# mandanasmi/lane-slam

Measured on AMD Instinct MI355X. Metric: frames/sec (640x480) detect->descript->project->sanity->associate, higher is better.
Workload: dtype u8/f64 (FP4 e2m1 MFMA with exact f32 accumulation for association)

## Files before the change

### include/lanefront.h

```cpp
#ifndef LANEFRONT_H
#define LANEFRONT_H

#include <stddef.h>
#include <stdint.h>

#define LF_API __attribute__((visibility("default")))

#ifdef __cplusplus
extern "C" {
#endif

#define LF_ABI_VERSION 5

typedef enum lf_status {
    LF_OK = 0,
    LF_ERR_BAD_ARG = -1,
    LF_ERR_CAPACITY = -2,
    LF_ERR_HIP = -3,
    LF_ERR_NOT_INITIALISED = -4,
    LF_ERR_UNSUPPORTED = -5,
    LF_ERR_DECODE = -6
} lf_status;

#define LF_WHITE 0
// ... 66 lines not shown
    double rho, theta;
} lf_hough_params;
LF_API void lf_hough_default_params(lf_hough_params* p);
LF_API int lf_set_hough_params(lf_handle* h, const lf_hough_params* p);
LF_API int lf_get_hough_params(const lf_handle* h, lf_hough_params* p);
#define LF_DETECTOR_DENSE 3
typedef struct lf_dense_params {
    double sobel_threshold;
} lf_dense_params;
LF_API void lf_dense_default_params(lf_dense_params* p);
LF_API int lf_set_dense_params(lf_handle* h, const lf_dense_params* p);
LF_API int lf_get_dense_params(const lf_handle* h, lf_dense_params* p);

#define LF_TIE_LOWEST 0
#define LF_TIE_MIHASHER 1
LF_API int lf_associate(lf_handle* h, const uint8_t* query32, int nq, const uint8_t* map32, int nm,
                 int32_t* idx, float* dist, int on_device);
LF_API int lf_set_tie_rule(lf_handle* h, int tie_rule);
LF_API int lf_associate_float(lf_handle* h, const float* query72, int nq, const float* map72, int nm,
                       int32_t* idx, float* dist, int on_device);

LF_API int lf_knn_match(lf_handle* h, const uint8_t* query32, int nq, const uint8_t* map32, int nm, int k, int32_t* idx, float* dist,
                 int on_device);
LF_API int lf_select_queries(lf_handle* h, const uint8_t* query32, int nq, const uint8_t* mask, uint8_t* selected32, int32_t* query_idx,
                      int* n_selected, int on_device);
LF_API int lf_radius_match(lf_handle* h, const uint8_t* query32, int nq, const uint8_t* map32, int nm, float max_distance,
                    int32_t* offsets, int32_t* idx, float* dist, int cap, int* total, int on_device);

typedef struct { int32_t queryIdx, trainIdx, imgIdx; float distance; } lf_dmatch;
LF_API int lf_matcher_add(lf_handle* h, const uint8_t* codes32, int n, int on_device);
LF_API int lf_matcher_clear(lf_handle* h);
LF_API int lf_matcher_size(const lf_handle* h, int* n_images, int* n_descriptors);
LF_API int lf_matcher_match(lf_handle* h, const uint8_t* query32, int nq, const uint8_t* const* masks, lf_dmatch* out, int* n_out);
LF_API int lf_matcher_knn_match(lf_handle* h, const uint8_t* query32, int nq, int k, const uint8_t* const* masks, int compact_result,
                         int32_t* list_offsets, lf_dmatch* out, int* n_lists);
LF_API int lf_matcher_radius_match(lf_handle* h, const uint8_t* query32, int nq, float max_distance, const uint8_t* const* masks,
                            int compact_result, int32_t* list_offsets, lf_dmatch* out, int cap, int* n_lists, int* total);

LF_API int lf_kmeans(lf_handle* h, const uint8_t* bgr_points, int n, int on_device, int k, const double* init_centers, int max_iter,
              double tol, double* centers_out, long long* counts_out, double* inertia_out, int* n_iter_out);

typedef struct lf_ai_transform {
    int32_t status;
    int32_t success;
    int32_t n_colors;
    int32_t n_iter3, n_iter4;
    int32_t reserved;
    double scale[3], shift[3];
    double cost, health;
    double score3, score4;
    double centers[3][3];
    int64_t counts[3];
} lf_ai_transform;
LF_API int lf_ai_transform_batch(lf_handle* h, const uint8_t* frames, int n_frames, int frames_on_device, int rows, int cols,
                                 lf_ai_transform* out);
LF_API int lf_set_ai_transform(lf_handle* h, const double scale[3], const double shift[3]);
LF_API int lf_get_ai_transform(const lf_handle* h, double scale[3], double shift[3]);

typedef struct lf_map lf_map;
#define LF_MAP_APPEND 0
#define LF_MAP_MERGE 1
#define LF_MAP_RING 0
#define LF_MAP_FULL_ERROR 1
#define LF_BLOCK_ROW_BYTES 80
typedef struct lf_map_config {
    int32_t capacity;
    int32_t color_gating;
    int32_t max_distance;
    int32_t policy;
    int32_t kept_only;
    int32_t merge_distance;
    int32_t when_full;
} lf_map_config;

LF_API int lf_map_create(int device_id, const lf_map_config* cfg, lf_map** out);
LF_API void lf_map_destroy(lf_map* m);
LF_API const char* lf_map_last_error(const lf_map* m);
LF_API int lf_map_get_stream(lf_map* m, void** hip_stream);
LF_API int lf_map_synchronize(lf_map* m);
LF_API int lf_map_seed(lf_map* m, const uint8_t* code32, const uint8_t* color, const double* ground4, int n, int on_device);
LF_API int lf_map_size(lf_map* m, int* size, int* head, int64_t* total_appended, int64_t* total_refreshed);
LF_API int lf_map_associate(lf_map* m, lf_handle* h, const uint8_t* code32, const uint8_t* color, int n,
                     int32_t* idx, float* dist, int on_device);
LF_API int lf_map_set_tie_rule(lf_map* m, int tie_rule);
LF_API int lf_map_pack_block(lf_map* m, lf_handle* h, const lf_segments* segs, int n, int n_frames, const int32_t* idx,
                      const float* dist, const double* frame_pose, int step, uint8_t* block, int block_rows);
LF_API int lf_map_update(lf_map* m, const uint8_t* blocks, int n_blocks, int block_rows);
LF_API int lf_map_step(lf_map* m, lf_handle* h, const lf_segments* segs, int n, int n_frames, const double* frame_pose,
                int step, int32_t* idx, float* dist);
LF_API int lf_map_step_host(lf_map* m, const lf_segments* segs, int n, int n_frames, const double* frame_pose, int step,
                     int32_t* idx, float* dist);
LF_API int lf_map_fetch(lf_map* m, int first, int n, uint8_t* code32, uint8_t* color, double* ground4, int32_t* hits,
                 int32_t* last_seen);

#define LF_MAP_N_STAGES 4
LF_API int lf_map_set_profiling(lf_map* m, int enabled);
LF_API int lf_map_get_timing(lf_map* m, double* ms_per_stage, int32_t* launches_per_stage, int n);
LF_API const char* lf_map_stage_name(int stage);

typedef struct lf_map_view {
    int32_t rows, cols;
    double  x_min, y_max;
    double  pixels_per_metre;
    int32_t thickness;
    int32_t min_hits;
    int32_t min_last_seen;
    uint32_t color_mask;
    uint8_t background[3];
    uint8_t pad_[1];
} lf_map_view;

LF_API void lf_map_default_view(lf_map_view* v);
LF_API int lf_map_bounds(lf_map* m, const lf_map_view* v, double* bounds4, int* n_entries);
LF_API int lf_map_render(lf_map* m, const lf_map_view* v, const double* trajectory, int n_points, uint8_t* out, int out_on_device,
                  int* n_drawn, int* n_skipped);
LF_API int lf_map_render_counts(lf_map* m, int* n_drawn, int* n_skipped);
#define LF_MAP_RENDER_STAGES 4
LF_API int lf_map_render_timing(lf_map* m, double* ms_per_stage, int n);
LF_API const char* lf_map_render_stage_name(int stage);

typedef struct lf_camera_view {
    int32_t rows, cols;
    int32_t top_cutoff;
    int32_t cam_w, cam_h;
    double  hinv[9];
    double  w_near;
    int32_t thickness;
    int32_t min_hits, min_last_seen;
    uint32_t color_mask;
    int32_t palette_size;
    uint8_t palette[8][3];
    uint8_t background[3];
    uint8_t pad_[1];
} lf_camera_view;
LF_API int lf_sizeof_camera_view(void);
LF_API int lf_map_camera_view(const double* H, int cam_w, int cam_h, int rows, int cols, int top_cutoff, lf_camera_view* v);
LF_API int lf_map_render_camera(lf_map* m, const lf_camera_view* v, const double* frame_pose, int n_frames, const uint8_t* src, uint8_t* out,
                         int on_device, int32_t* counts );
LF_API int lf_map_render_camera_timing(lf_map* m, double* ms_per_stage, int n);

typedef struct lf_align_config {
    int32_t iterations;
    int32_t min_pairs;
    int32_t min_hits;
    int32_t color_match;
    double  gate;
    double  huber;
    double  max_dist;
    double  prior_xy, prior_theta;
    double  max_shift, max_turn;
} lf_align_config;
typedef struct lf_align_result {
    double  x, y, theta;
    double  cost0, cost;
    int32_t n_pairs, n_used;
    int32_t iterations;
    int32_t status;
} lf_align_result;
enum { LF_ALIGN_OK = 0, LF_ALIGN_FEW = 1, LF_ALIGN_DEGENERATE = 2, LF_ALIGN_REJECTED = 3 };
LF_API int lf_sizeof_align_config(void);
LF_API int lf_sizeof_align_result(void);
LF_API void lf_map_align_default_config(lf_align_config* c);
LF_API int lf_map_align(lf_map* m, lf_handle* h, const lf_segments* segs, int n, int n_frames, const int32_t* idx, const float* dist,
                 const double* frame_pose , const lf_align_config* cfg, int on_device,
                 lf_align_result* results );
LF_API int lf_map_step_aligned(lf_map* m, lf_handle* h, const lf_segments* segs, int n, int n_frames, const double* frame_pose,
// ... 266 lines not shown
LF_API int lf_get_descriptor_params(lf_handle* h, lf_descriptor_params* p);
LF_API int lf_keylines_batch(lf_handle* h, const uint8_t* images, int n_frames, int input_kind, int images_on_device, int n_octaves,
                      const lf_edlines_params* params_or_null, lf_keylines* out, int out_on_device, int describe,
                      int* n_keylines, int32_t* frame_status_or_null);
LF_API int lf_keylines_batch_masked(lf_handle* h, const uint8_t* images, int n_frames, int input_kind, int images_on_device, int n_octaves,
                             const lf_edlines_params* params_or_null, const uint8_t* masks, int masks_on_device, lf_keylines* out,
                             int out_on_device, int describe, int* n_keylines, int32_t* frame_status);
LF_API int lf_keylines_batch_async(lf_handle* h, const uint8_t* images_dev, int n_frames, int input_kind, int n_octaves,
                            const lf_edlines_params* params_or_null, lf_keylines* out_dev, int describe);
LF_API int lf_keylines_frame_status(lf_handle* h, int32_t* frame_status, int n_frames);
LF_API int lf_lsd_keylines_batch(lf_handle* h, const uint8_t* images, int n_frames, int input_kind, int images_on_device, int n_octaves,
                          lf_keylines* out, int out_on_device, int describe, int* n_keylines);
typedef struct {
    int32_t refine;
    int32_t n_bins;
    double scale, sigma_scale, quant, ang_th, log_eps, density_th;
    double min_length;
} lf_lsd_options;
LF_API void lf_lsd_default_options(lf_lsd_options* opts);
LF_API int lf_lsd_keylines_batch_ex(lf_handle* h, const uint8_t* images, int n_frames, int input_kind, int images_on_device, int n_octaves,
                             const lf_lsd_options* opts, const uint8_t* masks, int masks_on_device,
                             lf_keylines* out, int out_on_device, int describe, int* n_keylines);
LF_API int lf_set_image_edlines(lf_handle* h, const uint8_t* bgr, int rows, int cols, int row_stride_bytes,
                         const lf_edlines_params* params_or_null);
LF_API int lf_describe_keylines(lf_handle* h, const uint8_t* gray, int n_frames, const int32_t* line_frame, const float* in_octave4,
                         const float* angle, const int32_t* num_pixels, const int32_t* octave, int n, float* desc72,
                         uint8_t* code32, int on_device);
LF_API int lf_keylines_debug_fetch(lf_handle* h, int octave, int what, void* dst, size_t bytes, int32_t* dims5_or_null);

LF_API int lf_jpeg_decode_batch(lf_handle* h, const uint8_t* const* jpeg, const size_t* jpeg_size, int n_frames,
                         int rows, int cols, uint8_t* frames, int frames_on_device, int n_threads,
                         int* frame_status);
LF_API int lf_jpeg_decode_batch_gpu(lf_handle* h, const uint8_t* const* jpeg, const size_t* jpeg_size, int n_frames,
                             int rows, int cols, uint8_t* frames, int frames_on_device, int n_threads,
                             int* frame_status);
LF_API int lf_jpeg_decode_batch_gpu_async(lf_handle* h, const uint8_t* const* jpeg, const size_t* jpeg_size, int n_frames,
                                   int rows, int cols, uint8_t* frames_device, int n_threads);
LF_API int lf_jpeg_status(lf_handle* h, int* frame_status, int n_frames, int* n_failed);
LF_API int lf_jpeg_decode_for_detect_async(lf_handle* h, const uint8_t* const* jpeg, const size_t* jpeg_size, int n_frames, int n_threads);
LF_API int lf_jpeg_info(const uint8_t* jpeg, size_t jpeg_size, int* rows, int* cols, int* components, int* hmax, int* vmax);
LF_API int lf_frames_buffer(lf_handle* h, uint8_t** device_ptr, size_t* bytes);

#define LF_MSG_DETECTOR 0
#define LF_MSG_GROUND 1
#define LF_MSG_FILTERED 2
LF_API int lf_serialize_segments(lf_handle* h, const lf_segments* segs, int segs_on_device, int n_frames, int stage,
                          uint8_t* out, size_t out_capacity, int out_on_device, int64_t* frame_byte_offset);
LF_API int lf_deserialize_segments(lf_handle* h, const uint8_t* bodies, int bodies_on_device, const int64_t* frame_byte_offset,
                            int n_frames, lf_segments* out, int out_on_device, int* n_segments);

LF_API int lf_draw_lines(lf_handle* h, int n_frames, const lf_segments* seg, int seg_on_device, uint8_t* out_bgr, int out_on_device);
LF_API int lf_draw_lines_image(lf_handle* h, const uint8_t* bgr, int n_frames, int rows, int cols, const lf_segments* seg, int seg_on_device,
                               uint8_t* out_bgr, int images_on_device);

#define LF_JPEG_ENCODE_STAGES 8
LF_API size_t lf_jpeg_encode_bound(int rows, int cols);
LF_API int lf_jpeg_encode_batch(lf_handle* h, const uint8_t* bgr, int bgr_on_device, int n_frames, int rows, int cols, int quality, uint8_t* out,
                                size_t out_stride, uint32_t* out_size, int out_on_device);
LF_API int lf_jpeg_encode_timing(lf_handle* h, double* ms_per_stage, int n);
LF_API const char* lf_jpeg_encode_stage_name(int stage);

#define LF_RECTIFY_STAGES 1
LF_API int lf_set_camera(lf_handle* h, const double* K, const double* D, const double* R, const double* P, int cam_w, int cam_h);
LF_API int lf_set_rectified_input(lf_handle* h, int flag);
LF_API int lf_get_rectified_input(lf_handle* h, int* flag);
LF_API int lf_rectify_map(lf_handle* h, float* mapx, float* mapy);
LF_API int lf_rectify_batch(lf_handle* h, const uint8_t* src, int src_on_device, int n_frames, int rows, int cols, int channels, uint8_t* dst,
                            int dst_on_device);
LF_API int lf_rectify_timing(lf_handle* h, double* ms_per_stage, int n);
LF_API const char* lf_rectify_stage_name(int stage);

typedef enum lf_buffer_id {
    LF_BUF_BGR = 0,
    LF_BUF_MASKS = 1,
    LF_BUF_EDGES = 2,
    LF_BUF_LSD_ANGLE = 3,
    LF_BUF_LSD_MODGRAD = 4,
    LF_BUF_LSD_ORDER = 5,
    LF_BUF_LSD_NORDER = 6,
    LF_BUF_LBD_DX = 7,
    LF_BUF_LBD_DY = 8,
    LF_BUF_LSD_COUNTS = 9,
    LF_BUF_LSD_SCRATCH = 10,
    LF_BUF_LSD_NLOW = 11
} lf_buffer_id;
LF_API int lf_debug_fetch(lf_handle* h, int buffer_id, void* dst, size_t bytes);
LF_API int lf_debug_detmath(lf_handle* h, int which, const double* a, const double* b_or_null, double* y, int n);
enum { LF_WAVE_INT = 0, LF_WAVE_UINT = 1, LF_WAVE_FLOAT = 2, LF_WAVE_DOUBLE = 3, LF_WAVE_LONG = 4, LF_WAVE_ULONG = 5 };
enum {
    LF_WAVE_READLANE = 0, LF_WAVE_DPP = 1, LF_WAVE_SUM = 2, LF_WAVE_MAX = 3, LF_WAVE_MIN = 4, LF_WAVE_INCL_SCAN_DPP = 5,
    LF_WAVE_INCL_MIN_DPP = 6, LF_WAVE_SUM_BCAST = 7, LF_WAVE_MIN_BCAST = 8, LF_WAVE_INCL_SCAN = 9, LF_WAVE_REDUCE = 10,
    LF_WAVE_BALLOT = 11, LF_WAVE_LANE_MASK_LT = 12, LF_WAVE_LANES_BELOW = 13, LF_WAVE_BALLOT_BRANCH = 14, LF_WAVE_UNI = 15,
    LF_WAVE_WG_EXCL_SCAN = 16, LF_WAVE_WG_SCAN_TURNS = 17
};
LF_API int lf_debug_wave(lf_handle* h, int op, int type, int arg, int diverge, const uint64_t* in, uint64_t* out, int n_threads, int block);
LF_API int lf_debug_probe(lf_handle* h, int width, int write, size_t bytes, int reps);
LF_API int lf_debug_lsd_binary(lf_handle* h, const uint8_t* img, int rows, int cols, float* lines4, int cap, int* n_out);
LF_API int lf_debug_hysteresis(lf_handle* h, const uint8_t* planes_u8, int n_frames, int rows, int cols, uint8_t* edges_u8_out);
LF_API int lf_debug_segments(lf_handle* h, int mode, int n_frames, const int32_t* counts, const float* lines4, const uint8_t* masks,
                             lf_segments* out, int* n_segments);
LF_API int lf_debug_std_sort(lf_handle* h, const int32_t* keys, int n, int32_t* order);
LF_API int lf_debug_assoc_plan(int nq, int nm, int32_t out[6]);
LF_API int lf_lsd_size(const lf_handle* h, int* rows, int* cols);
LF_API int lf_suggested_depth(const lf_handle* h);

LF_API int lf_lsd_list_capacity(const lf_handle* h, int* entries, int* grown);
LF_API int lf_lsd_scratch_stride(const lf_handle* h);

#define LF_N_STAGES 16
LF_API int lf_set_profiling(lf_handle* h, int enabled);
LF_API int lf_get_timing(lf_handle* h, double* ms_per_stage, int32_t* launches_per_stage, int n);
LF_API int lf_reset_timing(lf_handle* h);
LF_API const char* lf_stage_name(int stage);

#ifdef __cplusplus
}
#endif
#endif
```

### lane_slam_amd/_lib.py

```python
import ctypes
import os

from .config import LfConfig

_HERE = os.path.dirname(os.path.abspath(__file__))
SO_PATH = os.environ.get("LANEFRONT_LIBRARY") or os.path.join(_HERE, "liblanefront.so")

LF_N_STAGES = 16
LF_MAP_N_STAGES = 4
LF_MSG_DETECTOR, LF_MSG_GROUND, LF_MSG_FILTERED = 0, 1, 2
(LF_BUF_BGR, LF_BUF_MASKS, LF_BUF_EDGES, LF_BUF_LSD_ANGLE, LF_BUF_LSD_MODGRAD, LF_BUF_LSD_ORDER,
 LF_BUF_LSD_NORDER, LF_BUF_LBD_DX, LF_BUF_LBD_DY, LF_BUF_LSD_COUNTS, LF_BUF_LSD_SCRATCH, LF_BUF_LSD_NLOW) = range(12)

EXPORTS = (
    "lf_abi_version", "lf_create", "lf_destroy", "lf_last_error", "lf_synchronize", "lf_get_stream",
    "lf_set_image", "lf_detect_lines", "lf_process_batch", "lf_process_batch_async", "lf_wait", "lf_associate", "lf_associate_float", "lf_kmeans",
    "lf_jpeg_decode_batch", "lf_jpeg_info", "lf_frames_buffer", "lf_serialize_segments", "lf_deserialize_segments",
    "lf_debug_fetch", "lf_debug_detmath", "lf_debug_wave", "lf_debug_probe", "lf_debug_lsd_binary", "lf_debug_segments", "lf_debug_hysteresis", "lf_lsd_size", "lf_set_profiling", "lf_get_timing", "lf_reset_timing", "lf_stage_name",
    "lf_map_create", "lf_map_destroy", "lf_map_last_error", "lf_map_get_stream", "lf_map_synchronize", "lf_map_seed", "lf_map_size",
    "lf_map_associate", "lf_map_pack_block", "lf_map_update", "lf_map_step", "lf_map_step_host", "lf_map_fetch",
    "lf_map_set_profiling", "lf_map_get_timing", "lf_map_stage_name",
    "lf_descriptor_default_params", "lf_set_descriptor_params", "lf_get_descriptor_params",
    "lf_edlines_default_params", "lf_keylines_batch", "lf_describe_keylines", "lf_keylines_debug_fetch", "lf_set_image_edlines", "lf_knn_match", "lf_radius_match", "lf_jpeg_decode_batch_gpu", "lf_jpeg_decode_batch_gpu_async", "lf_jpeg_status", "lf_jpeg_decode_for_detect_async",
    "lf_set_tie_rule", "lf_map_set_tie_rule", "lf_debug_std_sort", "lf_debug_assoc_plan", "lf_suggested_depth", "lf_lsd_list_capacity", "lf_lsd_scratch_stride", "lf_set_detector", "lf_detector_failures", "lf_keylines_batch_async", "lf_keylines_frame_status", "lf_lsd_keylines_batch", "lf_select_queries",
    "lf_lsd_default_options", "lf_lsd_keylines_batch_ex", "lf_keylines_batch_masked",
    "lf_matcher_add", "lf_matcher_clear", "lf_matcher_size", "lf_matcher_match", "lf_matcher_knn_match", "lf_matcher_radius_match",
    "lf_lane_filter_default_config", "lf_lane_filter_create", "lf_lane_filter_destroy", "lf_lane_filter_last_error", "lf_lane_filter_grid",
    "lf_lane_filter_set_tables", "lf_lane_filter_reset", "lf_lane_filter_step", "lf_lane_filter_get_poses", "lf_lane_filter_get_belief",
    "lf_lane_filter_synchronize", "lf_lane_filter_set_profiling", "lf_lane_filter_get_timing", "lf_lane_filter_stage_name",
    "lf_hough_default_params", "lf_set_hough_params", "lf_get_hough_params",
    "lf_dense_default_params", "lf_set_dense_params", "lf_get_dense_params",
    "lf_ai_transform_batch", "lf_set_ai_transform", "lf_get_ai_transform",
    "lf_draw_lines", "lf_draw_lines_image",
    "lf_jpeg_encode_bound", "lf_jpeg_encode_batch", "lf_jpeg_encode_timing", "lf_jpeg_encode_stage_name",
    "lf_set_camera", "lf_set_rectified_input", "lf_get_rectified_input", "lf_rectify_map", "lf_rectify_batch", "lf_rectify_timing",
    "lf_rectify_stage_name",
    "lf_map_default_view", "lf_map_bounds", "lf_map_render", "lf_map_render_counts", "lf_map_render_timing", "lf_map_render_stage_name",
    "lf_sizeof_camera_view", "lf_map_camera_view", "lf_map_render_camera", "lf_map_render_camera_timing",
    "lf_sizeof_align_config", "lf_sizeof_align_result", "lf_map_align_default_config", "lf_map_align", "lf_map_step_aligned",
    "lf_map_step_aligned_host", "lf_map_align_timing",
    "lf_sizeof_smooth_config", "lf_map_smooth_default_config", "lf_map_smooth", "lf_map_step_smoothed", "lf_map_step_smoothed_host",
    "lf_map_smooth_timing",
    "lf_sizeof_localize_config", "lf_sizeof_localize_result", "lf_map_localize_default_config", "lf_map_localize", "lf_map_localize_timing",
    "lf_sizeof_prune_config", "lf_sizeof_prune_result", "lf_map_prune_default_config", "lf_map_prune", "lf_map_prune_timing",
    "lf_sizeof_near_config", "lf_map_near_default_config", "lf_map_associate_near", "lf_map_set_near", "lf_map_get_near", "lf_map_near_timing",
    "lf_sizeof_lanes_config", "lf_sizeof_lane", "lf_sizeof_lanes_result", "lf_map_lanes_default_config", "lf_map_lanes", "lf_map_lanes_timing",
    "lf_sizeof_polylines_config", "lf_sizeof_polyline_vertex", "lf_sizeof_polyline", "lf_sizeof_polylines_result",
    "lf_map_polylines_default_config", "lf_map_polylines", "lf_map_polylines_timing",
    "lf_sizeof_lane_pose_config", "lf_sizeof_lane_pose", "lf_sizeof_lane_pose_result",
    "lf_map_lane_pose_default_config", "lf_map_lane_pose", "lf_map_lane_pose_timing",
    "lf_sizeof_graph_config", "lf_sizeof_graph_result", "lf_map_graph_default_config", "lf_map_graph_solve", "lf_map_correct",
    "lf_map_graph_timing",
)
LF_ALIGN_OK, LF_ALIGN_FEW, LF_ALIGN_DEGENERATE, LF_ALIGN_REJECTED = 0, 1, 2, 3
ALIGN_STATUS = ("ok", "few", "degenerate", "rejected")
LF_MAP_RENDER_STAGES = 4
LF_JPEG_ENCODE_STAGES = 8
LF_RECTIFY_STAGES = 1
LF_LANE_FILTER_PREDICT, LF_LANE_FILTER_UPDATE = 1, 2
LF_LANE_FILTER_MAX_CELLS = 4096
LF_LANE_FILTER_N_STAGES = 2
LANE_FILTER_PARAMS = ("mean_d_0", "mean_phi_0", "sigma_d_0", "sigma_phi_0", "delta_d", "delta_phi", "d_max", "d_min", "phi_max",
                      "phi_min", "cov_v", "linewidth_white", "linewidth_yellow", "lanewidth", "min_max", "sigma_d_mask", "sigma_phi_mask")
DETECTORS = {"lsd": 0, "edlines": 1, "hough": 2, "dense": 3}
HOUGH_KEYS = ("hough_threshold", "hough_min_line_length", "hough_max_line_gap")
DENSE_KEYS = ("sobel_threshold",)
TIE_RULES = {"lowest": 0, "mihasher": 1}
LF_MAX_OCTAVES = 5


class LfSegments(ctypes.Structure):
    _fields_ = [
        ("capacity", ctypes.c_int32),
        ("frame_offset", ctypes.c_void_p),
        ("lines", ctypes.c_void_p), ("normals", ctypes.c_void_p), ("color", ctypes.c_void_p),
        ("pixels_normalized", ctypes.c_void_p), ("ground", ctypes.c_void_p), ("keep", ctypes.c_void_p),
        ("desc", ctypes.c_void_p), ("code", ctypes.c_void_p),
    ]


class LfEdlinesParams(ctypes.Structure):
    _fields_ = [("gradient_threshold", ctypes.c_int32), ("anchor_threshold", ctypes.c_int32), ("scan_intervals", ctypes.c_int32),
                ("min_line_len", ctypes.c_int32), ("line_fit_err_threshold", ctypes.c_double), ("ksize", ctypes.c_int32)]


class LfHoughParams(ctypes.Structure):
    _fields_ = [("threshold", ctypes.c_int32), ("min_line_length", ctypes.c_int32), ("max_line_gap", ctypes.c_int32),
                ("rho", ctypes.c_double), ("theta", ctypes.c_double)]


class LfDenseParams(ctypes.Structure):
    _fields_ = [("sobel_threshold", ctypes.c_double)]


class LfAiTransform(ctypes.Structure):
    _fields_ = [("status", ctypes.c_int32), ("success", ctypes.c_int32), ("n_colors", ctypes.c_int32), ("n_iter3", ctypes.c_int32),
                ("n_iter4", ctypes.c_int32), ("reserved", ctypes.c_int32), ("scale", ctypes.c_double * 3), ("shift", ctypes.c_double * 3),
                ("cost", ctypes.c_double), ("health", ctypes.c_double), ("score3", ctypes.c_double), ("score4", ctypes.c_double),
                ("centers", ctypes.c_double * 9), ("counts", ctypes.c_int64 * 3)]


class LfDescriptorParams(ctypes.Structure):
    _fields_ = [("num_of_octave", ctypes.c_int32), ("width_of_band", ctypes.c_int32), ("reduction_ratio", ctypes.c_int32), ("ksize", ctypes.c_int32)]

# ... 211 lines not shown
    lib.lf_get_ai_transform.argtypes = [vp, vp, vp]
    lib.lf_draw_lines.argtypes = [vp, ci, ctypes.POINTER(LfSegments), ci, vp, ci]
    lib.lf_draw_lines_image.argtypes = [vp, vp, ci, ci, ci, ctypes.POINTER(LfSegments), ci, vp, ci]
    lib.lf_jpeg_encode_bound.argtypes = [ci, ci]
    lib.lf_jpeg_encode_bound.restype = ctypes.c_size_t
    lib.lf_jpeg_encode_batch.argtypes = [vp, vp, ci, ci, ci, ci, ci, vp, ctypes.c_size_t, vp, ci]
    lib.lf_jpeg_encode_batch.restype = ci
    lib.lf_jpeg_encode_timing.argtypes = [vp, vp, ci]
    lib.lf_jpeg_encode_timing.restype = ci
    lib.lf_jpeg_encode_stage_name.argtypes = [ci]
    lib.lf_jpeg_encode_stage_name.restype = ctypes.c_char_p
    lib.lf_set_camera.argtypes = [vp, vp, vp, vp, vp, ci, ci]
    lib.lf_set_rectified_input.argtypes = [vp, ci]
    lib.lf_get_rectified_input.argtypes = [vp, ctypes.POINTER(ci)]
    lib.lf_rectify_map.argtypes = [vp, vp, vp]
    lib.lf_rectify_batch.argtypes = [vp, vp, ci, ci, ci, ci, ci, vp, ci]
    lib.lf_rectify_timing.argtypes = [vp, vp, ci]
    for f in ("lf_set_camera", "lf_set_rectified_input", "lf_get_rectified_input", "lf_rectify_map", "lf_rectify_batch", "lf_rectify_timing"):
        getattr(lib, f).restype = ci
    lib.lf_rectify_stage_name.argtypes = [ci]
    lib.lf_rectify_stage_name.restype = ctypes.c_char_p
    lib.lf_jpeg_decode_batch.argtypes = [vp, ctypes.POINTER(vp), ctypes.POINTER(ctypes.c_size_t), ci, ci, ci, vp, ci, ci,
                                         ctypes.POINTER(ci)]
    lib.lf_jpeg_decode_batch.restype = ci
    lib.lf_jpeg_decode_batch_gpu.argtypes = lib.lf_jpeg_decode_batch.argtypes
    lib.lf_jpeg_decode_batch_gpu.restype = ci
    lib.lf_jpeg_decode_batch_gpu_async.argtypes = [vp, ctypes.POINTER(vp), ctypes.POINTER(ctypes.c_size_t), ci, ci, ci, vp, ci]
    lib.lf_jpeg_decode_batch_gpu_async.restype = ci
    lib.lf_jpeg_status.argtypes = [vp, ctypes.POINTER(ci), ci, ctypes.POINTER(ci)]
    lib.lf_jpeg_decode_for_detect_async.argtypes = [vp, ctypes.POINTER(vp), ctypes.POINTER(ctypes.c_size_t), ci, ci]
    lib.lf_jpeg_decode_for_detect_async.restype = ci
    lib.lf_jpeg_status.restype = ci
    lib.lf_jpeg_info.argtypes = [vp, ctypes.c_size_t] + [ctypes.POINTER(ci)] * 5
    lib.lf_jpeg_info.restype = ci
    lib.lf_frames_buffer.argtypes = [vp, ctypes.POINTER(vp), ctypes.POINTER(ctypes.c_size_t)]
    lib.lf_frames_buffer.restype = ci
    lib.lf_serialize_segments.argtypes = [vp, ctypes.POINTER(LfSegments), ci, ci, ci, vp, ctypes.c_size_t, ci,
                                          ctypes.POINTER(ctypes.c_int64)]
    lib.lf_serialize_segments.restype = ci
    lib.lf_deserialize_segments.argtypes = [vp, vp, ci, ctypes.POINTER(ctypes.c_int64), ci, ctypes.POINTER(LfSegments), ci,
                                            ctypes.POINTER(ci)]
    lib.lf_deserialize_segments.restype = ci
    lib.lf_debug_fetch.argtypes = [vp, ci, vp, ctypes.c_size_t]
    lib.lf_debug_detmath.argtypes = [vp, ci, vp, vp, vp, ci]
    lib.lf_debug_detmath.restype = ci
    lib.lf_debug_wave.argtypes = [vp, ci, ci, ci, ci, vp, vp, ci, ci]
    lib.lf_debug_wave.restype = ci
    lib.lf_debug_probe.argtypes = [vp, ci, ci, ctypes.c_size_t, ci]
    lib.lf_debug_probe.restype = ci
    lib.lf_debug_lsd_binary.argtypes = [vp, vp, ci, ci, vp, ci, ctypes.POINTER(ci)]
    lib.lf_debug_lsd_binary.restype = ci
    lib.lf_debug_segments.argtypes = [vp, ci, ci, vp, vp, vp, ctypes.POINTER(LfSegments), ctypes.POINTER(ci)]
    lib.lf_debug_hysteresis.argtypes = [vp, vp, ci, ci, ci, vp]
    lib.lf_debug_hysteresis.restype = ci
    lib.lf_lsd_size.argtypes = [vp, ctypes.POINTER(ci), ctypes.POINTER(ci)]
    lib.lf_set_profiling.argtypes = [vp, ci]
    lib.lf_get_timing.argtypes = [vp, vp, vp, ci]
    lib.lf_reset_timing.argtypes = [vp]
    lib.lf_stage_name.argtypes = [ci]
    lib.lf_stage_name.restype = ctypes.c_char_p
    i64p = ctypes.POINTER(ctypes.c_int64)
    lib.lf_map_create.argtypes = [ci, ctypes.POINTER(LfMapConfig), ctypes.POINTER(vp)]
    lib.lf_map_destroy.argtypes = [vp]
    lib.lf_map_destroy.restype = None
    lib.lf_map_last_error.argtypes = [vp]
    lib.lf_map_last_error.restype = ctypes.c_char_p
    lib.lf_map_get_stream.argtypes = [vp, ctypes.POINTER(vp)]
    lib.lf_map_synchronize.argtypes = [vp]
    lib.lf_map_seed.argtypes = [vp, vp, vp, vp, ci, ci]
    lib.lf_map_size.argtypes = [vp, ctypes.POINTER(ci), ctypes.POINTER(ci), i64p, i64p]
    lib.lf_map_associate.argtypes = [vp, vp, vp, vp, ci, vp, vp, ci]
    lib.lf_map_pack_block.argtypes = [vp, vp, ctypes.POINTER(LfSegments), ci, ci, vp, vp, vp, ci, vp, ci]
    lib.lf_map_update.argtypes = [vp, vp, ci, ci]
    lib.lf_map_step.argtypes = [vp, vp, ctypes.POINTER(LfSegments), ci, ci, vp, ci, vp, vp]
    lib.lf_map_step_host.argtypes = [vp, ctypes.POINTER(LfSegments), ci, ci, vp, ci, vp, vp]
    lib.lf_map_step_host.restype = ci
    lib.lf_map_fetch.argtypes = [vp, ci, ci, vp, vp, vp, vp, vp]
    lib.lf_map_set_profiling.argtypes = [vp, ci]
    lib.lf_map_set_profiling.restype = ci
    lib.lf_map_get_timing.argtypes = [vp, vp, vp, ci]
    lib.lf_map_get_timing.restype = ci
    lib.lf_map_stage_name.argtypes = [ci]
    lib.lf_map_stage_name.restype = ctypes.c_char_p
    lib.lf_map_default_view.argtypes = [ctypes.POINTER(LfMapView)]
    lib.lf_map_default_view.restype = None
    lib.lf_map_bounds.argtypes = [vp, ctypes.POINTER(LfMapView), vp, ctypes.POINTER(ci)]
    lib.lf_map_render.argtypes = [vp, ctypes.POINTER(LfMapView), vp, ci, vp, ci, ctypes.POINTER(ci), ctypes.POINTER(ci)]
    lib.lf_map_render_counts.argtypes = [vp, ctypes.POINTER(ci), ctypes.POINTER(ci)]
    lib.lf_map_render_timing.argtypes = [vp, vp, ci]
    for f in ("lf_map_bounds", "lf_map_render", "lf_map_render_counts", "lf_map_render_timing"):
        getattr(lib, f).restype = ci
    lib.lf_map_render_stage_name.argtypes = [ci]
    lib.lf_map_render_stage_name.restype = ctypes.c_char_p
    lib.lf_sizeof_camera_view.argtypes = []
    lib.lf_map_camera_view.argtypes = [vp, ci, ci, ci, ci, ci, ctypes.POINTER(LfCameraView)]
    lib.lf_map_render_camera.argtypes = [vp, ctypes.POINTER(LfCameraView), vp, ci, vp, vp, ci, vp]
    lib.lf_map_render_camera_timing.argtypes = [vp, vp, ci]
    for f in ("lf_sizeof_camera_view", "lf_map_camera_view", "lf_map_render_camera", "lf_map_render_camera_timing"):
        getattr(lib, f).restype = ci
    lib.lf_sizeof_align_config.argtypes = []
    lib.lf_sizeof_align_result.argtypes = []
    lib.lf_map_align_default_config.argtypes = [ctypes.POINTER(LfAlignConfig)]
    lib.lf_map_align_default_config.restype = None
    lib.lf_map_align.argtypes = [vp, vp, ctypes.POINTER(LfSegments), ci, ci, vp, vp, vp, ctypes.POINTER(LfAlignConfig), ci, vp]
    lib.lf_map_step_aligned.argtypes = [vp, vp, ctypes.POINTER(LfSegments), ci, ci, vp, ctypes.POINTER(LfAlignConfig), ci, vp, vp, vp]
    lib.lf_map_step_aligned_host.argtypes = [vp, ctypes.POINTER(LfSegments), ci, ci, vp, ctypes.POINTER(LfAlignConfig), ci, vp, vp, vp]
    lib.lf_map_align_timing.argtypes = [vp, ctypes.POINTER(ctypes.c_double), ctypes.POINTER(ctypes.c_int32)]
    for f in ("lf_sizeof_align_config", "lf_sizeof_align_result", "lf_map_align", "lf_map_step_aligned", "lf_map_step_aligned_host",
              "lf_map_align_timing"):
        getattr(lib, f).restype = ci
    lib.lf_sizeof_smooth_config.argtypes = []
    lib.lf_map_smooth_default_config.argtypes = [ctypes.POINTER(LfSmoothConfig)]
    lib.lf_map_smooth_default_config.restype = None
    lib.lf_map_smooth.argtypes = [vp, vp, ctypes.POINTER(LfSegments), ci, ci, vp, vp, vp, vp, ci, ctypes.POINTER(LfSmoothConfig), ci, vp, vp]
    lib.lf_map_step_smoothed.argtypes = [vp, vp, ctypes.POINTER(LfSegments), ci, ci, vp, vp, ci, ctypes.POINTER(LfSmoothConfig), ci, vp, vp, vp, vp]
    lib.lf_map_step_smoothed_host.argtypes = [vp, ctypes.POINTER(LfSegments), ci, ci, vp, vp, ci, ctypes.POINTER(LfSmoothConfig), ci, vp, vp, vp, vp]
    lib.lf_map_smooth_timing.argtypes = [vp, ctypes.POINTER(ctypes.c_double), ctypes.POINTER(ctypes.c_int32)]
    for f in ("lf_sizeof_smooth_config", "lf_map_smooth", "lf_map_step_smoothed", "lf_map_step_smoothed_host", "lf_map_smooth_timing"):
        getattr(lib, f).restype = ci
    lib.lf_sizeof_localize_config.argtypes = []
    lib.lf_sizeof_localize_result.argtypes = []
    lib.lf_map_localize_default_config.argtypes = [ctypes.POINTER(LfLocalizeConfig)]
    lib.lf_map_localize_default_config.restype = None
    lib.lf_map_localize.argtypes = [vp, vp, ctypes.POINTER(LfSegments), ci, ci, vp, vp, vp, ctypes.POINTER(LfLocalizeConfig), ci, vp]
    lib.lf_map_localize_timing.argtypes = [vp, ctypes.POINTER(ctypes.c_double), ctypes.POINTER(ctypes.c_int32)]
    for f in ("lf_sizeof_localize_config", "lf_sizeof_localize_result", "lf_map_localize", "lf_map_localize_timing"):
        getattr(lib, f).restype = ci
    lib.lf_sizeof_prune_config.argtypes = []
    lib.lf_sizeof_prune_result.argtypes = []
    lib.lf_map_prune_default_config.argtypes = [ctypes.POINTER(LfPruneConfig)]
    lib.lf_map_prune_default_config.restype = None
    lib.lf_map_prune.argtypes = [vp, ctypes.POINTER(LfPruneConfig), ctypes.POINTER(LfPruneResult), vp, ci]
    lib.lf_map_prune_timing.argtypes = [vp, ctypes.POINTER(ctypes.c_double), ctypes.POINTER(ctypes.c_int32)]
    for f in ("lf_sizeof_prune_config", "lf_sizeof_prune_result", "lf_map_prune", "lf_map_prune_timing"):
        getattr(lib, f).restype = ci
    lib.lf_sizeof_near_config.argtypes = []
    lib.lf_map_near_default_config.argtypes = [ctypes.POINTER(LfNearConfig)]
    lib.lf_map_near_default_config.restype = None
    lib.lf_map_associate_near.argtypes = [vp, vp, ctypes.POINTER(LfSegments), ci, ci, vp, ctypes.POINTER(LfNearConfig), vp, vp, vp, ci]
    lib.lf_map_set_near.argtypes = [vp, ctypes.POINTER(LfNearConfig)]
    lib.lf_map_get_near.argtypes = [vp, ctypes.POINTER(LfNearConfig)]
    lib.lf_map_near_timing.argtypes = [vp, ctypes.POINTER(ctypes.c_double), ctypes.POINTER(ctypes.c_int32)]
    for f in ("lf_sizeof_near_config", "lf_map_associate_near", "lf_map_set_near", "lf_map_get_near", "lf_map_near_timing"):
        getattr(lib, f).restype = ci
    for f in ("lf_sizeof_lanes_config", "lf_sizeof_lane", "lf_sizeof_lanes_result"):
        getattr(lib, f).argtypes = []
    lib.lf_map_lanes_default_config.argtypes = [ctypes.POINTER(LfLanesConfig)]
    lib.lf_map_lanes_default_config.restype = None
    lib.lf_map_lanes.argtypes = [vp, ctypes.POINTER(LfLanesConfig), ctypes.POINTER(LfLanesResult), vp, vp, vp, vp, ci, ci]
    lib.lf_map_lanes_timing.argtypes = [vp, ctypes.POINTER(ctypes.c_double), ctypes.POINTER(ctypes.c_int32)]
    for f in ("lf_sizeof_lanes_config", "lf_sizeof_lane", "lf_sizeof_lanes_result", "lf_map_lanes", "lf_map_lanes_timing"):
        getattr(lib, f).restype = ci
    for f in ("lf_sizeof_polylines_config", "lf_sizeof_polyline_vertex", "lf_sizeof_polyline", "lf_sizeof_polylines_result"):
        getattr(lib, f).argtypes = []
        getattr(lib, f).restype = ci
    lib.lf_map_polylines_default_config.argtypes = [ctypes.POINTER(LfPolylinesConfig)]
    lib.lf_map_polylines_default_config.restype = None
    lib.lf_map_polylines.argtypes = [vp, ctypes.POINTER(LfPolylinesConfig), ctypes.POINTER(LfPolylinesResult), vp, vp, ci, vp, ci, ci]
    lib.lf_map_polylines.restype = ci
    lib.lf_map_polylines_timing.argtypes = [vp, ctypes.POINTER(ctypes.c_double), ctypes.POINTER(ctypes.c_int32)]
    lib.lf_map_polylines_timing.restype = ci
    for f in ("lf_sizeof_lane_pose_config", "lf_sizeof_lane_pose", "lf_sizeof_lane_pose_result"):
        getattr(lib, f).argtypes = []
        getattr(lib, f).restype = ci
    lib.lf_map_lane_pose_default_config.argtypes = [ctypes.POINTER(LfLanePoseConfig)]
    lib.lf_map_lane_pose_default_config.restype = None
# ... 120 lines not shown
```

### lane_slam_amd/csrc/common.h

```cpp
#pragma once
#include <hip/hip_runtime.h>
#include <stdint.h>
#include <stddef.h>
#include "../../include/lanefront.h"
#include "detmath.h"

namespace lf {

constexpr int kMaxKsize = 9;
constexpr int kMaxGaussTaps = 15;
constexpr float kNotDef = -1024.0f;
#ifndef LF_LABEL_ITEMS
#define LF_LABEL_ITEMS 8192
#endif
constexpr int kLabelItems = LF_LABEL_ITEMS;
#ifndef LF_LABEL_LDS
#define LF_LABEL_LDS 6144
#endif
constexpr int kLabelLds = LF_LABEL_LDS;
constexpr int kCompCap = 1024;

enum Stage {
    ST_PRE = 0, ST_CANNY, ST_HYST, ST_LSD_GRAD, ST_LSD_ORDER, ST_LSD_GROW, ST_SEGMENTS,
    ST_LBD_GRAD, ST_LBD, ST_ASSOC_PACK, ST_ASSOC, ST_MISC, ST_JPEG, ST_LSD_LABEL, ST_HOUGH, ST_DENSE, ST_COUNT
// ... 223 lines not shown
{
    *reinterpret_cast<uint32_t*>(mx + assoc_map_offset_fp4(pos, 4 * b)) = 0u;
    if (b < 8) *reinterpret_cast<uint32_t*>(mcx + pos * 32 + 4 * b) = 0u;
}
#endif
template <typename T>
struct DevArray {
    T* p = nullptr;
    size_t bytes = 0;
    DevArray() = default;
    DevArray(DevArray&& o) noexcept : p(o.p), bytes(o.bytes) { o.p = nullptr; o.bytes = 0; }
    DevArray& operator=(DevArray&& o) noexcept
    {
        if (this != &o) { reset(); p = o.p; bytes = o.bytes; o.p = nullptr; o.bytes = 0; }
        return *this;
    }
    ~DevArray() { reset(); }
    hipError_t alloc(size_t n_bytes)
    {
        reset();
        const hipError_t e = hipMalloc((void**)&p, n_bytes);
        if (e != hipSuccess) p = nullptr; else bytes = n_bytes;
        return e;
    }
    void reset() { if (p) (void)hipFree(p); p = nullptr; bytes = 0; }
    operator T*() const { return p; }
};
using DevBuf = DevArray<void>;

template <typename T>
struct HostArray {
    T* p = nullptr;
    size_t bytes = 0;
    HostArray() = default;
    HostArray(HostArray&& o) noexcept : p(o.p), bytes(o.bytes) { o.p = nullptr; o.bytes = 0; }
    HostArray& operator=(HostArray&& o) noexcept
    {
        if (this != &o) { reset(); p = o.p; bytes = o.bytes; o.p = nullptr; o.bytes = 0; }
        return *this;
    }
    ~HostArray() { reset(); }
    hipError_t alloc(size_t n_bytes)
    {
        reset();
        const hipError_t e = hipHostMalloc((void**)&p, n_bytes, hipHostMallocDefault);
        if (e != hipSuccess) p = nullptr; else bytes = n_bytes;
        return e;
    }
    void reset() { if (p) (void)hipHostFree(p); p = nullptr; bytes = 0; }
    operator T*() const { return p; }
};

struct AssocScratch {
    DevArray<unsigned int> part; DevArray<int> done; size_t cap_part = 0, cap_blocks = 0;
    int qblocks = 0, splits = 0, m_chunk = 0;
    DevArray<int> tie_list; size_t cap_list = 0;
    unsigned long long* tie_res = nullptr;
};
void launch_assoc_pack_map(const uint8_t* codes, int n, int n_pad, int8_t* x, hipStream_t s);
hipError_t launch_assoc_core(const uint8_t* q, const uint8_t* qcolor, int nq, const int8_t* mx, const int8_t* mcx, int nm,
                             const int* nm_dev, int gating, int max_distance, AssocScratch& w, int32_t* idx, float* dist, hipStream_t s);
hipError_t launch_assoc_ties(const uint8_t* q, const uint8_t* qcolor, int nq, const int8_t* mx, const uint8_t* mcode, const uint8_t* mcolor,
                             int nm, const int* nm_dev, int gating, AssocScratch& w, unsigned long long* res, int32_t* idx, const float* dist, hipStream_t s);
hipError_t launch_assoc(const uint8_t* q, int nq, const uint8_t* m, int nm, int8_t* mx, AssocScratch& w, int32_t* idx, float* dist, hipStream_t s);
void launch_assoc_nomatch(int nq, int32_t* idx, float* dist, hipStream_t s);
void launch_kmeans(const uint8_t* bgr, int n, int k, const double* init, int max_iter, double tol_rel, uint8_t* lab, double* out,
                   long long* counts, int* status, hipStream_t s);
void launch_draw(const void* src, bool src_bgrx, uint8_t* out, int n_frames, int Hc, int W, const int32_t* frame_offset, const float* lines,
                 const uint8_t* color, int capacity, int* bad, hipStream_t s);
void launch_ai_transform(const uint8_t* strips, long long frame_stride, int n_frames, int S, int cols, uint8_t* lab, double* fo,
                         long long* fc, int* fs, lf_ai_transform* out, hipStream_t s);
struct MapDevice {
    int capacity, policy, kept_only, merge_distance, when_full;
    uint8_t* code; uint8_t* color; double* ground; int* hits; int* last_seen; int* winner;
    int8_t* mx; int8_t* mcx;
    int* state;
    unsigned long long* totals;
};
void launch_fill_i32(int* p, size_t n, int v, hipStream_t s);
void launch_map_pack_block(int n, int n_frames, const int* frame_offset, const uint8_t* code, const uint8_t* color,
                           const uint8_t* keep, const double* ground, const int32_t* idx, const float* dist,
                           const double* pose4, int step, uint8_t* block, hipStream_t s);
void launch_map_overflow_block(int n, int n_frames, int step, uint8_t* block, hipStream_t s);
void launch_map_seed_block(int n, const uint8_t* code, const uint8_t* color, const double* ground, uint8_t* block, hipStream_t s);
void launch_map_update(const MapDevice& md, const uint8_t* blocks, int n_blocks, int block_rows, int force_append, int* act,
                       hipStream_t s);
void launch_select_queries(const uint8_t* q, const uint8_t* mask, int nq, uint8_t* out, int32_t* qidx, int* n_out, hipStream_t s);
void launch_knn(const uint8_t* q, int nq, const uint8_t* m, int nm, int k, int max_distance, int mih, int32_t* idx, float* dist, hipStream_t s);
void launch_radius(const uint8_t* q, int nq, const uint8_t* m, int nm, int max_distance, int32_t* hist, int32_t* count, int32_t* offsets,
                   int* total, int cap, int mih, int32_t* idx, float* dist, hipStream_t s);
size_t assoc_float_scratch_bytes(int nq, int nm);
hipError_t launch_assoc_float(const float* q, int nq, const float* m, int nm, float* qn, float* mn,
                              void* scratch, int32_t* idx, float* dist, hipStream_t s);
namespace jpeg { struct FrameHeader; }
struct JpegGeom { int rows, cols, Wp, Hp; int first_row = 0; };
void launch_jpeg_decode(const JpegGeom& g, int n_frames, int max_blocks, const jpeg::FrameHeader* hdrs,
                        const uint32_t* entries, const uint32_t* block_end, uint8_t* planes, uint8_t* frames,
                        hipStream_t s);

void launch_jpeg_color(const JpegGeom& g, int n_frames, const void* hdrs, size_t hdr_stride, const uint8_t* planes, uint8_t* frames, hipStream_t s);
namespace jpeg { struct DevFrame; }
void launch_jh_decode(const JpegGeom& g, int n_frames, int max_blocks, size_t max_scan_len, jpeg::DevFrame* frames, const uint8_t* bytes, uint8_t* clean,
                      uint32_t* seg_begin, void* info, uint32_t* sub, int16_t* coef, int* status, uint8_t* planes, hipStream_t s);
size_t jh_info_bytes();

void launch_msg_layout(int n_frames, int stage, const int* frame_offset, const uint8_t* keep, int* counts,
                       long long* byte_offset, hipStream_t s);
void launch_msg_write(int n_frames, int stage, const int* frame_offset, const uint8_t* color, const float* pixels_normalized,
                      const float* normals, const double* ground, const uint8_t* keep, const int* counts,
                      const long long* byte_offset, uint8_t* out, hipStream_t s);
void launch_msg_read(int n_frames, int capacity, const uint8_t* body, const long long* byte_offset, int* frame_offset,
                     int* bad, uint8_t* color, float* pixels_normalized, float* normals, double* ground, hipStream_t s);

}
```

### lane_slam_amd/csrc/k_lsd_order.hip

```cpp
#include <cstdlib>
#include <algorithm>
#include "common.h"
#include <type_traits>
#include "lsd_bitplane.h"
#include "scan.h"
#include "wave.h"

namespace lf {
using std::max;
using std::min;

#ifndef LF_ORDER_THREADS
#define LF_ORDER_THREADS 512
#endif
#ifndef LF_ORDER_BM_THREADS
#define LF_ORDER_BM_THREADS 256
#endif
#ifndef LF_LABEL_THREADS
#define LF_LABEL_THREADS 256
#endif
constexpr int OT = LF_ORDER_THREADS;
constexpr int OBT = LF_ORDER_BM_THREADS;
constexpr int NB = 16;
constexpr int LDS_ITEMS = 8192;
// ... 501 lines not shown
        __syncthreads();
    } else {
        for (int e = t; e < n; e += LT) reinterpret_cast<uint16_t*>(dyn_lds + LS / 2)[e] = (uint16_t)(c_xy[o + e] & 0xffffu);
        __syncthreads();
    for (int e = t; e < n; e += LT) {
        const int y = (int)(c_xy[o + e] >> 16);
        const int first = rs[y];
        int h = e;
        int xh = xs(h);
        while (h > first) { const int xp = xs(h - 1); if (xp + 1 != xh) break; --h; xh = xp; }
        parent.set((uint32_t)e, (uint32_t)h);
    }
    __syncthreads();
    for (int e = t; e < n; e += LT) {
        const uint32_t xy = c_xy[o + e];
        const int x = (int)(xy & 0xffffu), y = (int)(xy >> 16);
        if (y > 0) {
            int lo = rs[y - 1];
            const int end = rs[y];
            int hi = end;
            while (lo < hi) { const int mid = (lo + hi) >> 1; if (xs(mid) < x - 1) lo = mid + 1; else hi = mid; }
            for (int k = lo; k < end && k < lo + 3 && xs(k) <= x + 1; ++k) uf_unite(parent, (uint32_t)e, (uint32_t)k);
        }
    }
    __syncthreads();
    }
    for (int i = t; i < (n + 1) / 2; i += LT) csize2.set((uint32_t)i, 0u);
    __syncthreads();
    for (int e = t; e < n; e += LT) {
        const uint32_t r = uf_find(parent, (uint32_t)e);
        lab[e] = (uint16_t)r;
        csize2.add(r >> 1, 1u << (16 * (r & 1u)));
    }
    __syncthreads();
    auto csize = [&](uint32_t r) -> uint32_t { return (csize2.get(r >> 1) >> (16 * (r & 1u))) & 0xffffu; };
    const uint32_t minsz = p.min_reg_size > 1 ? (uint32_t)p.min_reg_size : 1u;
    for (int e = t; e < n; e += LT)
        if (csize((uint32_t)e) >= minsz) {
            const int k = atomicAdd(&n_roots, 1);
            if (k < comp_cap) roots[k] = (uint16_t)e;
        }
    __syncthreads();
    const int C = n_roots;
    if (C > comp_cap) {
        for (int e = t; e < n; e += LT) lab[e] = 0;
        if (t == 0) { list[0] = 0; comp_count[pc] = 1; comp_key[pc] = n; }
        return;
    }
    for (int i = t; i < C; i += LT) {
        const uint32_t ri = roots[i], si = csize(ri);
        int rank = 0;
        for (int j = 0; j < C; ++j) {
            const uint32_t rj = roots[j], sj = csize(rj);
            rank += (sj > si || (sj == si && rj < ri)) ? 1 : 0;
        }
        list[rank] = (uint16_t)ri;
        parent.set(ri, (uint32_t)rank);
        if (rank == 0) comp_key[pc] = (int)si;
        if (rank >= kCompTop) atomicAdd(&rest_total, (int)si);
    }
    __syncthreads();
    if (C <= kCompTop) {
        if (t == 0) { comp_count[pc] = C; if (C == 0) comp_key[pc] = 0; }
        return;
    }
    __threadfence_block();
    const uint16_t rest_root = list[kCompTop];
    for (int e = t; e < n; e += LT) {
        const uint32_t r = lab[e];
        if (csize(r) >= minsz && parent.get(r) >= (uint32_t)kCompTop) lab[e] = rest_root;
    }
    if (t == 0) {
        const int rest = rest_total;
        const int top0 = (int)csize((uint32_t)list[0]);
        if (rest > top0) {
            for (int k = kCompTop; k > 0; --k) list[k] = list[k - 1];
            list[0] = rest_root;
            comp_key[pc] = rest;
        }
        comp_count[pc] = kCompTop + 1;
    }
}

__global__ __launch_bounds__(256) void k_lsd_rank(int n_prob, const int* __restrict__ norder, int* __restrict__ perm)
{
    __shared__ int nd[1024];
    if (n_prob > 1024) {
        for (int i = threadIdx.x; i < n_prob; i += 256) perm[i] = i;
        return;
    }
    for (int i = threadIdx.x; i < n_prob; i += 256) nd[i] = norder[i];
    __syncthreads();
    for (int i = threadIdx.x; i < n_prob; i += 256) {
        const int mine = nd[i];
        int rank = 0;
        for (int j = 0; j < n_prob; ++j) rank += (nd[j] > mine || (nd[j] == mine && j < i)) ? 1 : 0;
        perm[rank] = i;
    }
}

void launch_lsd_rank(const LsdComponents& m, int n_prob, hipStream_t s)
{
    hipLaunchKernelGGL(k_lsd_rank, dim3(1), dim3(256), 0, s, n_prob, m.comp_key, m.perm);
}

__global__ __launch_bounds__(LT) void k_lsd_label(LsdParams p, const int* __restrict__ norder, const uint32_t* __restrict__ c_xy,
                                                  const int* __restrict__ row_start, uint16_t* __restrict__ c_label,
                                                  uint16_t* __restrict__ comp_list, int* __restrict__ comp_count, int* __restrict__ comp_key, int comp_cap,
                                                  uint32_t* __restrict__ scratch, size_t scratch_stride, int plane_fits)
{
    const int n = norder[blockIdx.x];
    if (n <= p.label_lds)
        lsd_label_problem<false>(p, norder, c_xy, row_start, c_label, comp_list, comp_count, comp_key, comp_cap, scratch, scratch_stride);
    else if (plane_fits)
        lsd_label_problem<true>(p, norder, c_xy, row_start, c_label, comp_list, comp_count, comp_key, comp_cap, scratch, scratch_stride);
    else {
        const size_t o = (size_t)blockIdx.x * p.rec_cap;
        for (int e = threadIdx.x; e < n; e += LT) c_label[o + e] = 0;
        if (threadIdx.x == 0) { comp_list[(size_t)blockIdx.x * kCompCap] = 0; comp_count[blockIdx.x] = 1; comp_key[blockIdx.x] = n; }
    }
}

void launch_lsd_label(const LsdParams& p, const LsdCompact& c, const LsdComponents& m, int n_frames, hipStream_t s)
{
    size_t lds = (size_t)p.label_lds * (2 + 2);
    const size_t plane = bitplane_lds_words((size_t)p.Hs * p.Ws) * 4;
    const int plane_fits = plane <= 150 * 1024 ? 1 : 0;
    if (plane_fits && plane > lds) lds = plane;
    if (lds > 48 * 1024)
        (void)hipFuncSetAttribute(reinterpret_cast<const void*>(k_lsd_label), hipFuncAttributeMaxDynamicSharedMemorySize, (int)lds);
    static const int comp_cap = getenv("LF_DIAG_COMP_CAP") ? max(1, min(kCompCap, atoi(getenv("LF_DIAG_COMP_CAP")))) : kCompCap;
    const size_t stride = lsd_grow_reg_stride(p);
    hipLaunchKernelGGL(k_lsd_label, dim3(n_frames * 3), dim3(LT), lds, s, p, c.norder, c.c_xy, c.row_start, m.c_label, m.comp_list, m.comp_count,
                       m.comp_key, comp_cap, m.reg, stride, plane_fits);
}

__global__ void k_lsd_dense_debug(LsdParams p, const int* __restrict__ norder, const uint32_t* __restrict__ c_xy,
                                  const float* __restrict__ c_deg, const double* __restrict__ c_mod,
                                  float* __restrict__ ang, double* __restrict__ mod)
{
    const int pc = blockIdx.x;
    const size_t Ps = (size_t)p.Hs * p.Ws, o = (size_t)pc * Ps, oc = (size_t)pc * p.rec_cap;
    for (size_t i = threadIdx.x; i < Ps; i += blockDim.x) { ang[o + i] = kNotDef; mod[o + i] = 0.0; }
    __syncthreads();
    const int n = norder[pc];
    for (int e = threadIdx.x; e < n; e += blockDim.x) {
        const uint32_t xy = c_xy[oc + e];
        const size_t a = (size_t)(xy >> 16) * p.Ws + (xy & 0xffffu);
        ang[o + a] = c_deg[oc + e];
        mod[o + a] = c_mod[oc + e];
    }
}

void launch_lsd_dense_debug(const LsdParams& p, const LsdCompact& c, int n_frames, float* ang, double* mod, hipStream_t s)
{
    hipLaunchKernelGGL(k_lsd_dense_debug, dim3(n_frames * 3), dim3(1024), 0, s, p, c.norder, c.c_xy, c.c_deg, c.c_mod, ang, mod);
}

}
```

### lane_slam_amd/csrc/k_map.hip

```cpp
#include "common.h"
#include "scan.h"

namespace lf {

constexpr int kRow = LF_BLOCK_ROW_BYTES;
constexpr int kRefFlag = 0x40000000;
constexpr uint32_t kMagic = 0x4b42464cu;

struct MapDev {
    int capacity, policy, kept_only, merge_distance, when_full;
    uint8_t* code; uint8_t* color; double* ground; int* hits; int* last_seen; int* winner;
    int8_t* mx; int8_t* mcx;
    int* state;
    unsigned long long* totals;
};

__global__ void k_map_pack_block(int n, int n_frames, const int* __restrict__ frame_offset, const uint8_t* __restrict__ code,
                                 const uint8_t* __restrict__ color, const uint8_t* __restrict__ keep,
                                 const double* __restrict__ ground, const int32_t* __restrict__ idx,
                                 const float* __restrict__ dist, const double* __restrict__ pose4, int step,
                                 uint8_t* __restrict__ block)
{
    const int s = blockIdx.x * blockDim.x + threadIdx.x;
    if (s == 0) {
// ... 126 lines not shown
    const int s = (int)(t >> 5), b = (int)(t & 31);
    if ((size_t)s >= total) return;
    int a = act[s];
    if (a == -1) return;
    if (!(a & kRefFlag)) a += wg_base[s / kMapWg];
    const int n_app = m.state[3], head0 = m.state[5], size0 = m.state[6], step = m.state[7];
    const int cap = m.capacity;
    int pos;
    bool fresh;
    if (a & kRefFlag) {
        pos = a & ~kRefFlag;
        if (m.winner[pos] != s) return;
        bool overwritten = false;
        if (m.when_full == LF_MAP_RING) {
            int rel = pos - head0; if (rel < 0) rel += cap;
            overwritten = n_app >= cap || rel < n_app;
        }
        if (overwritten) { if (b == 0) m.winner[pos] = -1; return; }
        fresh = false;
    } else {
        if (m.when_full == LF_MAP_RING) {
            if (n_app > cap && a < n_app - cap) return;
            pos = (int)(((long long)head0 + a) % cap);
        } else {
            if (a >= cap - size0) return;
            pos = size0 + a;
        }
        fresh = true;
    }
    const int blk = s / G, r = s - blk * G;
    const uint8_t* row = blocks + ((size_t)blk * block_rows + 1 + r) * kRow;
    const uint32_t byte = row[b];
    m.code[(size_t)pos * 32 + b] = (uint8_t)byte;
    assoc_map_write_row(m.mx, m.mcx, (size_t)pos, b, byte, row + 72);
    if (b == 0) {
        m.color[pos] = row[72];
        const double* rg = reinterpret_cast<const double*>(row + 32);
        for (int k = 0; k < 4; ++k) m.ground[(size_t)pos * 4 + k] = rg[k];
        m.last_seen[pos] = step;
        if (fresh) m.hits[pos] = 1; else m.winner[pos] = -1;
    }
}

__global__ void k_map_seed_block(int n, const uint8_t* __restrict__ code, const uint8_t* __restrict__ color,
                                 const double* __restrict__ ground, uint8_t* __restrict__ block)
{
    const int s = blockIdx.x * blockDim.x + threadIdx.x;
    if (s == 0) {
        uint32_t* hd = reinterpret_cast<uint32_t*>(block);
        hd[0] = kMagic; hd[1] = (uint32_t)n; hd[2] = (uint32_t)-1; hd[3] = 0u;
        for (int k = 4; k < kRow / 4; ++k) hd[k] = 0u;
    }
    if (s >= n) return;
    uint8_t* row = block + (size_t)(1 + s) * kRow;
    for (int k = 0; k < 32; ++k) row[k] = code[(size_t)s * 32 + k];
    double* rg = reinterpret_cast<double*>(row + 32);
    for (int k = 0; k < 4; ++k) rg[k] = ground ? ground[(size_t)s * 4 + k] : 0.0;
    *reinterpret_cast<int32_t*>(row + 64) = -1;
    *reinterpret_cast<float*>(row + 68) = -1.f;
    row[72] = color ? color[s] : (uint8_t)255;
    row[73] = 1;
    row[74] = row[75] = row[76] = row[77] = row[78] = row[79] = 0;
}

__global__ void k_fill_i32(int* p, size_t n, int v)
{
    for (size_t i = blockIdx.x * (size_t)blockDim.x + threadIdx.x; i < n; i += (size_t)gridDim.x * blockDim.x) p[i] = v;
}

void launch_fill_i32(int* p, size_t n, int v, hipStream_t s)
{
    if (n) hipLaunchKernelGGL(k_fill_i32, dim3(1024), dim3(256), 0, s, p, n, v);
}

void launch_map_pack_block(int n, int n_frames, const int* frame_offset, const uint8_t* code, const uint8_t* color,
                           const uint8_t* keep, const double* ground, const int32_t* idx, const float* dist,
                           const double* pose4, int step, uint8_t* block, hipStream_t s)
{
    const int threads = n > 0 ? n : 1;
    hipLaunchKernelGGL(k_map_pack_block, dim3((threads + 255) / 256), dim3(256), 0, s, n, n_frames, frame_offset, code, color,
                       keep, ground, idx, dist, pose4, step, block);
}

__global__ void k_map_overflow_block(int n, int n_frames, int step, uint8_t* __restrict__ block)
{
    uint32_t* hd = reinterpret_cast<uint32_t*>(block);
    const int k = threadIdx.x;
    if (k < kRow / 4) hd[k] = k == 0 ? kMagic : k == 2 ? (uint32_t)step : k == 3 ? (uint32_t)n_frames : k == 4 ? (uint32_t)n : 0u;
}

void launch_map_overflow_block(int n, int n_frames, int step, uint8_t* block, hipStream_t s)
{
    hipLaunchKernelGGL(k_map_overflow_block, dim3(1), dim3(64), 0, s, n, n_frames, step, block);
}

void launch_map_seed_block(int n, const uint8_t* code, const uint8_t* color, const double* ground, uint8_t* block, hipStream_t s)
{
    const int threads = n > 0 ? n : 1;
    hipLaunchKernelGGL(k_map_seed_block, dim3((threads + 255) / 256), dim3(256), 0, s, n, code, color, ground, block);
}

void launch_map_update(const MapDevice& md, const uint8_t* blocks, int n_blocks, int block_rows, int force_append, int* act,
                       hipStream_t s)
{
    MapDev m;
    m.capacity = md.capacity; m.policy = md.policy; m.kept_only = md.kept_only; m.merge_distance = md.merge_distance;
    m.when_full = md.when_full;
    m.code = md.code; m.color = md.color; m.ground = md.ground; m.hits = md.hits; m.last_seen = md.last_seen;
    m.winner = md.winner; m.mx = md.mx; m.mcx = md.mcx; m.state = md.state; m.totals = md.totals;
    const size_t rows = (size_t)n_blocks * (block_rows - 1);
    const int n_wg = (int)((rows + kMapWg - 1) / kMapWg);
    int* wg_count = act + rows;
    if (n_wg)
        hipLaunchKernelGGL(k_map_classify, dim3(n_wg), dim3(kMapWg), 0, s, m, blocks, n_blocks, block_rows, force_append, act, wg_count);
    hipLaunchKernelGGL(k_map_plan, dim3(1), dim3(kMapWg), 0, s, m, blocks, n_blocks, n_wg, wg_count);
    const size_t threads = rows * 32;
    if (threads)
        hipLaunchKernelGGL(k_map_apply, dim3((threads + 255) / 256), dim3(256), 0, s, m, blocks, n_blocks, block_rows, act, wg_count);
}

}
```

### lane_slam_amd/csrc/lanefront_api.hip

```cpp
#include <stdarg.h>
#include <stdio.h>
#include <string.h>
#include <math.h>
#include <vector>
#include <new>
#include <cstdlib>
#include "lanefront_handle.h"

using namespace lf;

static const char* kStageNames[LF_N_STAGES] = {
    "pre(resize+correct+hsv+masks+dilate)", "canny_nms", "canny_hysteresis", "lsd_blur_resample_grad",
    "lsd_order", "lsd_grow", "segments(normal+project+sanity)", "lbd_gray_blur_sobel", "lbd_descriptor",
    "assoc_pack", "assoc_mfma", "misc", "jpeg(idct+upsample+color)", "lsd_label(components+launch order)",
    "hough(probabilistic lines)", "dense(sobel-vote lines)" };

extern "C" void lf_set_error(lf_handle* h, int code, const char* fmt, ...)
{
    va_list ap;
    va_start(ap, fmt);
    vset_error(h, code, fmt, ap);
    va_end(ap);
}

static char g_create_err[512] = "no error";

static int cv_round_host(double v) { return dm::round_half_even(v); }

static int build_params(lf_handle* h)
{
    const lf_config& c = h->cfg;
    h->Hc = c.img_rows - c.top_cutoff;
    h->W = c.img_cols;
    if (h->Hc <= 0 || h->W <= 0 || c.in_rows <= 0 || c.in_cols <= 0 || c.top_cutoff < 0) {
        lf_set_error(h, LF_ERR_BAD_ARG, "bad geometry: in %dx%d img %dx%d cutoff %d", c.in_rows, c.in_cols, c.img_rows,
                     c.img_cols, c.top_cutoff);
        return LF_ERR_BAD_ARG;
    }
    if (h->W % 32 != 0) { lf_set_error(h, LF_ERR_UNSUPPORTED, "img_cols must be a multiple of 32 (got %d)", h->W); return LF_ERR_UNSUPPORTED; }
    h->P = (size_t)h->Hc * h->W;
    h->Ww = (h->W + 31) / 32;
    PreParams& p = h->pre;
    memset(&p, 0, sizeof(p));
    p.in_rows = c.in_rows; p.in_cols = c.in_cols; p.img_rows = c.img_rows; p.img_cols = c.img_cols;
    p.top_cutoff = c.top_cutoff; p.Hc = h->Hc; p.W = h->W;
    p.resize = (c.img_rows != c.in_rows) || (c.img_cols != c.in_cols);
    const double fx = (double)c.img_cols / (double)c.in_cols, fy = (double)c.img_rows / (double)c.in_rows;
    p.ifx = 1.0 / fx; p.ify = 1.0 / fy;
    p.identity_ai = 1;
    for (int i = 0; i < 3; ++i) { p.ai_scale[i] = c.ai_scale[i]; p.ai_shift[i] = c.ai_shift[i]; if (c.ai_scale[i] != 1.f || c.ai_shift[i] != 0.f) p.identity_ai = 0; }
    for (int k = 0; k < 4; ++k) for (int ch = 0; ch < 3; ++ch) { p.lo[k][ch] = c.hsv_lo[k][ch]; p.hi[k][ch] = c.hsv_hi[k][ch]; }
    p.ksize = c.dilation_kernel_size;
    if (p.ksize < 1 || p.ksize > kMaxKsize) { lf_set_error(h, LF_ERR_UNSUPPORTED, "dilation_kernel_size %d not in [1,%d]", p.ksize, kMaxKsize); return LF_ERR_UNSUPPORTED; }
    p.r = p.ksize / 2;
    {
        int r = p.ksize / 2, cc = p.ksize / 2;
        double inv_r2 = r ? 1.0 / ((double)r * r) : 0.0;
        for (int i = 0; i < p.ksize; ++i) {
            int dy = i - r;
            p.j1[i] = 0; p.j2[i] = 0;
            if (abs(dy) <= r) {
                int dx = cv_round_host(cc * sqrt((r * r - dy * dy) * inv_r2));
                p.j1[i] = cc - dx > 0 ? cc - dx : 0;
                p.j2[i] = cc + dx + 1 < p.ksize ? cc + dx + 1 : p.ksize;
            }
        }
        if (p.ksize % 2 == 0) { lf_set_error(h, LF_ERR_UNSUPPORTED, "even dilation kernels are not supported"); return LF_ERR_UNSUPPORTED; }
    }
    h->canny.Hc = h->Hc; h->canny.W = h->W; h->canny.Ww = h->Ww;
    double lo = c.canny_lo, hi = c.canny_hi;
    if (lo > hi) { double t = lo; lo = hi; hi = t; }
    h->canny.low = dm::ifloor(lo); h->canny.high = dm::ifloor(hi);
    if ((size_t)h->Hc * h->Ww > 8 * 1024 && (8192 / h->Ww < 1 || (int)((60 * 1024 / 4) / (2 * (size_t)h->Ww)) - 1 < 1)) { lf_set_error(h, LF_ERR_UNSUPPORTED, "img_cols %d: one row of the edge bit planes exceeds the hysteresis strip budget", h->W); return LF_ERR_UNSUPPORTED; }
    SegParams& S = h->seg;
    memset(&S, 0, sizeof(S));
    S.Hc = h->Hc; S.W = h->W; S.img_rows = c.img_rows; S.img_cols = c.img_cols; S.top_cutoff = c.top_cutoff;
    S.cap_lines = h->cap_lines;
    S.rx = 1.0 / (double)c.img_cols; S.ry = 1.0 / (double)c.img_rows; S.cut = (double)c.top_cutoff;
    memcpy(S.H, c.H, sizeof(S.H));
    seg_camera(h);
    S.lanewidth = c.lanewidth; S.linewidth_white = c.linewidth_white; S.linewidth_yellow = c.linewidth_yellow;
    S.d_min = c.d_min; S.d_max = c.d_max; S.phi_min = c.phi_min; S.phi_max = c.phi_max;
    return LF_OK;
}

static int lbd_weights(lf_handle* h, int w)
// ... 198 lines not shown
            return LF_ERR_UNSUPPORTED;
        }
    }
    if (h->detector == LF_DETECTOR_HOUGH) {
        int rc = hough_prepare(h);
        if (rc != LF_OK) return rc;
        StageClock::Scope t(h, h->clock, ST_HOUGH);
        LF_HIP_CHECK(h, hipMemsetAsync(h->lsd.d_zero, 0, h->lsd.zero_bytes, s));
        HoughParams hp = h->hough_p;
        hp.threshold = h->hough_params.threshold; hp.line_length = h->hough_params.min_line_length; hp.line_gap = h->hough_params.max_line_gap;
        launch_hough(hp, n * 3, h->hough_slots < n * 3 ? h->hough_slots : n * 3, h->d_strong, h->d_maskbits, h->d_hough_tab, h->d_hough_acc,
                     h->d_hough_nz, h->d_slot_lines, h->d_counts, s);
        LF_HIP_CHECK(h, hipGetLastError());
        h->slot_mode = SEG_HOUGH;
        h->last_frames = n;
        h->overflow_zeroed = true;
        return LF_OK;
    }
    if (dense) {
        StageClock::Scope t(h, h->clock, ST_DENSE);
        LF_HIP_CHECK(h, hipMemsetAsync(h->lsd.d_zero, 0, h->lsd.zero_bytes, s));
        launch_dense(h->Hc, h->W, h->Ww, h->cap_lines, (float)h->dense_params.sobel_threshold, n * 3, h->d_strong, h->d_maskbits,
                     h->d_bwbits, h->d_slot_lines, h->d_dense_rec, h->d_counts, s);
        LF_HIP_CHECK(h, hipGetLastError());
        h->slot_mode = SEG_DENSE;
        h->last_frames = n;
        h->overflow_zeroed = true;
        return LF_OK;
    }
    h->slot_mode = SEG_FLOAT;
    {
        StageClock::Scope t(h, h->clock, ST_LSD_GRAD);
        LF_HIP_CHECK(h, hipMemsetAsync(h->lsd.d_zero, 0, h->lsd.zero_bytes, s));
        h->lsd.grad(n, h->d_strong, h->d_maskbits, true, s);
    }
    { StageClock::Scope t(h, h->clock, ST_LSD_ORDER); h->lsd.order(n, 0, s); }
    {
        StageClock::Scope t(h, h->clock, ST_LSD_LABEL);
        h->lsd.label(n, true, s);
    }
    static const char* diag_skip = getenv("LF_DIAG_SKIP");
    if (diag_skip && strstr(diag_skip, "grow")) LF_HIP_CHECK(h, hipMemsetAsync(h->d_counts, 0, (size_t)n * 3 * sizeof(int), s));
    else {
        StageClock::Scope t(h, h->clock, ST_LSD_GROW);
        const LsdState& L = h->lsd;
        h->lsd.grow(n, h->d_slot_lines, h->d_counts, kGrowLdsKb[L.env_lds_level >= 0 ? L.env_lds_level : L.grow_lds_level],
                    L.env_mixed >= 0 ? L.env_mixed != 0 : L.grow_mixed, true, s);
    }
    LF_HIP_CHECK(h, hipGetLastError());
    h->last_frames = n;
    h->overflow_zeroed = true;
    return LF_OK;
}

int lf::run_segments(lf_handle* h, int n, lf_segments dev_out, bool describe)
{
    hipStream_t s = h->stream;
    {
        StageClock::Scope t(h, h->clock, ST_SEGMENTS);
        if (!h->overflow_zeroed) LF_HIP_CHECK(h, hipMemsetAsync(h->lsd.d_status, 0, offsetof(BatchStatus, detector_failures), s));
        h->overflow_zeroed = false;
        launch_seg_offsets(n, h->cap_lines, h->d_counts, h->d_seg_offset, dev_out.frame_offset ? dev_out.frame_offset : h->d_frame_offset,
                           h->lsd.d_status, h->slot_mode != SEG_FLOAT ? nullptr : h->lsd.d_norder, lsd_grow_def_lds(h->lsd.params, kGrowLdsKb[0]),
                           lsd_grow_def_lds(h->lsd.params, kGrowLdsKb[1]), s);
        launch_segments(h->seg, n, h->d_slot_lines, h->d_counts, h->d_seg_offset,
                        h->slot_mode == SEG_DENSE ? reinterpret_cast<const uint32_t*>(h->d_dense_rec.p) : h->d_maskbits.p, h->Ww, dev_out,
                        h->d_seg_frame, h->d_normals64, h->d_centers, s, h->slot_mode);
    }
    if (describe) {
        { StageClock::Scope t(h, h->clock, ST_LBD_GRAD); launch_lbd_grad(h->Hc, h->W, n, h->d_gray, h->d_dxy, s); }
        {
            StageClock::Scope t(h, h->clock, ST_LBD);
            int cap = dev_out.capacity < n * 3 * h->cap_lines ? dev_out.capacity : n * 3 * h->cap_lines;
            launch_lbd(h->Hc, h->W, cap, h->d_seg_offset + n * 3, dev_out.lines, h->d_seg_frame, h->d_dxy,
                       h->d_gauss_g, h->d_gauss_l, dev_out.desc, dev_out.code, s, h->desc_params.width_of_band);
        }
    }
    LF_HIP_CHECK(h, hipGetLastError());
    return LF_OK;
}

static int fetch_status(lf_handle* h) { LF_HIP_CHECK(h, hipMemcpyAsync(h->h_status, h->lsd.d_status, sizeof(BatchStatus), hipMemcpyDeviceToHost, h->stream)); return LF_OK; }

extern "C" int lf_process_batch_async(lf_handle* h, const uint8_t* frames, int n_frames, int frames_on_device,
                                      lf_segments* out_dev, int describe)
{
    if (!h) return LF_ERR_NOT_INITIALISED;
    if (!frames || !out_dev || n_frames < 1) { lf_set_error(h, LF_ERR_BAD_ARG, "lf_process_batch: null argument or n_frames < 1"); return LF_ERR_BAD_ARG; }
    if (n_frames > h->max_frames) { lf_set_error(h, LF_ERR_CAPACITY, "n_frames %d exceeds max_frames %d", n_frames, h->max_frames); return LF_ERR_CAPACITY; }
    if (describe && (!out_dev->lines)) { lf_set_error(h, LF_ERR_BAD_ARG, "describe needs out->lines"); return LF_ERR_BAD_ARG; }
    if (h->flight.kind != InFlight::NONE) { lf_set_error(h, LF_ERR_BAD_ARG, "a batch is already in flight on this handle: call lf_wait first"); return LF_ERR_BAD_ARG; }
    LF_HIP_CHECK(h, hipSetDevice(h->device));
    hipStream_t s = h->stream;
    const size_t frame_bytes = (size_t)h->cfg.in_rows * h->cfg.in_cols * 3;
    const uint8_t* d_in = frames;
    if (!frames_on_device) {
        int r0 = h->cfg.top_cutoff;
        if (h->pre.resize) r0 = dm::ifloor(h->cfg.top_cutoff * h->pre.ify) - 1;
        r0 = r0 < 0 ? 0 : (r0 > h->cfg.in_rows - 1 ? h->cfg.in_rows - 1 : r0);
        const size_t skip = (size_t)r0 * h->cfg.in_cols * 3;
        LF_HIP_CHECK(h, hipMemcpy2DAsync(h->d_frames + skip, frame_bytes, frames + skip, frame_bytes, frame_bytes - skip, (size_t)n_frames,
                                         hipMemcpyHostToDevice, s));
        d_in = h->d_frames;
    }
    h->plugin_ready = false;
    int rc = h->detector == LF_DETECTOR_EDLINES ? run_detect_edlines(h, d_in, n_frames) : run_detect(h, d_in, n_frames, false);
    if (rc != LF_OK) return rc;
    rc = run_segments(h, n_frames, *out_dev, describe != 0);
    if (rc != LF_OK || (rc = fetch_status(h)) != LF_OK) return rc;
    h->flight = InFlight{ InFlight::SEGMENTS, d_in, n_frames, *out_dev, describe != 0, n_frames * 3, out_dev->capacity };
    return LF_OK;
}

template <typename Copies>
static int detect_until_fit(lf_handle* h, const uint8_t* d_in, int n, bool from_working_image, const lf_segments& dev, bool describe, bool queued, Copies copies)
{
    const bool lists_used = from_working_image || h->detector != LF_DETECTOR_EDLINES;
    for (int attempt = 0;; ++attempt) {
        if (!queued) {
            int rc = run_detect(h, d_in, n, from_working_image);
            if (rc == LF_OK) rc = run_segments(h, n, dev, describe);
            if (rc == LF_OK) rc = copies();
            if (rc != LF_OK) return rc;
            LF_HIP_CHECK(h, hipStreamSynchronize(h->stream));
        }
        queued = false;
        const int need = h->h_status.p->rec_need;
        if (!lists_used || need <= h->lsd.params.rec_cap) return LF_OK;
        if (attempt == 4) { lf_set_error(h, LF_ERR_CAPACITY, "the LSD lists keep overflowing (%d entries needed)", need); return LF_ERR_CAPACITY; }
        if (const int rc = h->lsd.grow_lists(h, need)) return rc;
    }
}

extern "C" int lf_wait(lf_handle* h, int* n_segments)
{
    if (!h) return LF_ERR_NOT_INITIALISED;
    LF_HIP_CHECK(h, hipSetDevice(h->device));
    LF_HIP_CHECK(h, hipStreamSynchronize(h->stream));
    const InFlight f = h->flight;
    h->flight = InFlight{};
    switch (f.kind) {
    case InFlight::NONE: if (n_segments) *n_segments = 0; return LF_OK;
    case InFlight::KEYLINES: {
        const KlTotals t = h->kl ? *h->kl->batch.h_pinned : KlTotals{};
        if (n_segments) *n_segments = t.total;
        if (t.overflow) { lf_set_error(h, LF_ERR_CAPACITY, "%d KeyLines exceed the output capacity %d", t.total, f.capacity); return LF_ERR_CAPACITY; }
        return LF_OK;
    }
    case InFlight::SEGMENTS: break;
    }
    if (const int rc = detect_until_fit(h, f.in, f.n, false, f.out, f.describe, true, [h] { return fetch_status(h); })) return rc;
    const BatchStatus& st = *h->h_status;
    h->detector_failures = h->detector == LF_DETECTOR_EDLINES ? st.detector_failures : 0;
    h->draw_frames = 0;
    const int total = st.total;
    if (n_segments) *n_segments = total;
    h->lsd.adapt_slice(st.over_small, st.over_medium, f.problems);
    if (st.lines_overflow) { lf_set_error(h, LF_ERR_CAPACITY, "%s %s run produced more than max_lines_per_color=%d lines", h->detector == LF_DETECTOR_DENSE ? "a" : "an", detector_name(h->detector), h->cap_lines); return LF_ERR_CAPACITY; }
    if (total > f.capacity) { lf_set_error(h, LF_ERR_CAPACITY, "%d segments exceed the output capacity %d", total, f.capacity); return LF_ERR_CAPACITY; }
    h->draw_frames = f.n;
    return LF_OK;
}

extern "C" int lf_process_batch(lf_handle* h, const uint8_t* frames, int n_frames, int frames_on_device,
                                lf_segments* out, int out_on_device, int describe, int* n_segments)
{
    if (!h) return LF_ERR_NOT_INITIALISED;
    if (!out) { lf_set_error(h, LF_ERR_BAD_ARG, "lf_process_batch: null out"); return LF_ERR_BAD_ARG; }
    lf_segments dev = out_on_device ? *out : h->d_out;
    if (!out_on_device) {
        dev.capacity = out->capacity < h->out_capacity ? out->capacity : h->out_capacity;
        if (!out->normals) dev.normals = nullptr;
        if (!out->color) dev.color = nullptr;
        if (!out->pixels_normalized) dev.pixels_normalized = nullptr;
        if (!out->ground) dev.ground = nullptr;
        if (!out->keep) dev.keep = nullptr;
        if (!out->desc) dev.desc = nullptr;
        if (!out->code) dev.code = nullptr;
        dev.frame_offset = h->d_frame_offset;
        if (describe && !out->lines) { lf_set_error(h, LF_ERR_BAD_ARG, "describe needs out->lines"); return LF_ERR_BAD_ARG; }
    }
    int rc = lf_process_batch_async(h, frames, n_frames, frames_on_device, &dev, describe);
    if (rc != LF_OK) return rc;
    int total = 0;
    rc = lf_wait(h, &total);
    if (n_segments) *n_segments = total;
    if (rc != LF_OK) return rc;
    if (out_on_device) return LF_OK;
// ... 160 lines not shown
```

### lane_slam_amd/csrc/lanefront_core.h

```cpp
#pragma once
#include <stdarg.h>
#include <stdio.h>
#include <initializer_list>
#include <vector>
#include "common.h"

namespace lf {

struct Core {
    int device = 0;
    hipStream_t stream = nullptr;
    char err[512] = "";
    int err_code = 0;
    bool profiling = false;
};

inline void vset_error(Core* c, int code, const char* fmt, va_list ap)
{
    if (!c) return;
    vsnprintf(c->err, sizeof(c->err), fmt, ap);
    c->err_code = code;
}

__attribute__((format(printf, 3, 4))) inline void set_error(Core* c, int code, const char* fmt, ...)
// ... 18 lines not shown
    int ndev = 0;
    const hipError_t e = hipGetDeviceCount(&ndev);
    if (e != hipSuccess || ndev <= 0) {
        snprintf(buf, size, "%s: no HIP device (%s); lanefront has no CPU fallback", who, e != hipSuccess ? hipGetErrorString(e) : "device count 0");
        return LF_ERR_HIP;
    }
    if (device_id < 0 || device_id >= ndev) { snprintf(buf, size, "%s: device %d out of range (%d devices)", who, device_id, ndev); return LF_ERR_BAD_ARG; }
    return LF_OK;
}

template <typename T>
inline int scratch(Core* c, DevArray<T>& b, size_t bytes)
{
    if (b.bytes >= bytes) return LF_OK;
    if (b.p) { LF_HIP_CHECK(c, hipStreamSynchronize(c->stream)); b.reset(); }
    LF_HIP_CHECK(c, b.alloc(bytes + bytes / 4 + 256));
    return LF_OK;
}

struct Fetch { void* dst; const void* src; size_t bytes; };

inline int fetch(Core* c, std::initializer_list<Fetch> list)
{
    bool queued = false;
    for (const Fetch& f : list) {
        if (!f.dst || !f.src || !f.bytes || f.dst == f.src) continue;
        LF_HIP_CHECK(c, hipMemcpyAsync(f.dst, f.src, f.bytes, hipMemcpyDeviceToHost, c->stream));
        queued = true;
    }
    if (queued) LF_HIP_CHECK(c, hipStreamSynchronize(c->stream));
    return LF_OK;
}

struct Staging {
    explicit Staging(Core* c) : c_(c) {}

    template <typename T, typename B>
    const T* in(int on_device, const T* src, size_t bytes, DevArray<B>& buf, size_t room = 0)
    {
        if (on_device) return src;
        grow(buf, bytes > room ? bytes : room);
        if (bytes) up_.push_back({ buf.p, src, bytes });
        return static_cast<const T*>(static_cast<const void*>(buf.p));
    }

    template <typename T, typename B>
    T* in(int on_device, T* src, size_t bytes, DevArray<B>& buf, size_t room = 0)
    {
        return const_cast<T*>(in(on_device, static_cast<const T*>(src), bytes, buf, room));
    }

    template <typename T, typename B>
    T* out(int on_device, T* dst, size_t bytes, DevArray<B>& buf)
    {
        if (on_device) return dst;
        grow(buf, bytes);
        return static_cast<T*>(static_cast<void*>(buf.p));
    }

    int upload()
    {
        if (rc_ != LF_OK) return rc_;
        for (const Up& u : up_) LF_HIP_CHECK(c_, hipMemcpyAsync(u.dst, u.src, u.bytes, hipMemcpyHostToDevice, c_->stream));
        up_.clear();
        return LF_OK;
    }

private:
    struct Up { void* dst; const void* src; size_t bytes; };
    Core* c_;
    std::vector<Up> up_;
    int rc_ = LF_OK;

    template <typename B>
    void grow(DevArray<B>& buf, size_t bytes) { if (rc_ == LF_OK) rc_ = scratch(c_, buf, bytes); }
};

inline int stream_after(Core* c, hipEvent_t ev, hipStream_t waits, hipStream_t on)
{
    LF_HIP_CHECK(c, hipEventRecord(ev, on));
    LF_HIP_CHECK(c, hipStreamWaitEvent(waits, ev, 0));
    return LF_OK;
}

struct StageClock {
    struct Rec { hipEvent_t a, b; int st; };
    std::vector<double> ms;
    std::vector<int32_t> launches;

    StageClock(int n_stages, size_t cap, bool resolve_when_full) : ms(n_stages, 0.0), launches(n_stages, 0), cap_(cap), resolve_when_full_(resolve_when_full) {}
    StageClock(const StageClock&) = delete;
    StageClock& operator=(const StageClock&) = delete;
    ~StageClock()
    {
        for (std::vector<Rec>* v : { &used_, &free_ })
            for (Rec& r : *v) { (void)hipEventDestroy(r.a); (void)hipEventDestroy(r.b); }
    }

    void prefill(size_t n)
    {
        Rec r;
        while (free_.size() < n && make(&r)) free_.push_back(r);
    }

    void resolve()
    {
        for (Rec& r : used_) {
            (void)hipEventSynchronize(r.b);
            float t = 0;
            if (hipEventElapsedTime(&t, r.a, r.b) == hipSuccess) ms[r.st] += t;
            free_.push_back(r);
        }
        used_.clear();
    }

    void take(double* ms_out, int32_t* launches_out, int n, int first = 0, int count = -1)
    {
        resolve();
        const int end = count < 0 ? (int)ms.size() : first + count;
        for (int i = first; i < end; ++i) {
            if (i - first < n && ms_out) ms_out[i - first] = ms[i];
            if (i - first < n && launches_out) launches_out[i - first] = launches[i];
            ms[i] = 0; launches[i] = 0;
        }
    }

    struct Scope {
        Core* c; StageClock* k; int st; Rec r; bool on;
        Scope(Core* c_, StageClock& k_, int st_) : c(c_), k(&k_), st(st_), on(c_->profiling && k_.acquire(&r))
        {
            if (on) { r.st = st; (void)hipEventRecord(r.a, c->stream); }
        }
        Scope(const Scope&) = delete;
        Scope& operator=(const Scope&) = delete;
        ~Scope()
        {
            if (on) { (void)hipEventRecord(r.b, c->stream); k->used_.push_back(r); }
            k->launches[st] += 1;
        }
    };

private:
    std::vector<Rec> free_, used_;
    size_t cap_;
    bool resolve_when_full_;

    static bool make(Rec* r)
    {
        r->st = 0;
        if (hipEventCreate(&r->a) != hipSuccess) return false;
        if (hipEventCreate(&r->b) != hipSuccess) { (void)hipEventDestroy(r->a); return false; }
        return true;
    }
    bool acquire(Rec* r)
    {
        if (free_.empty()) {
            if (used_.size() >= cap_) {
                if (!resolve_when_full_) return false;
                resolve();
            } else {
                Rec n;
                if (!make(&n)) return false;
                free_.push_back(n);
            }
        }
        *r = free_.back(); free_.pop_back();
// ... 51 lines not shown
```

### lane_slam_amd/csrc/lanefront_debug.hip

```cpp
#include <string.h>
#include <vector>
#include "lanefront_handle.h"

using namespace lf;

extern "C" int lf_debug_std_sort(lf_handle* h, const int32_t* keys, int n, int32_t* order)
{
    if (!h) return LF_ERR_NOT_INITIALISED;
    if (!keys || !order || n < 1 || n >= (1 << 20)) { lf_set_error(h, LF_ERR_BAD_ARG, "lf_debug_std_sort: bad argument (1 <= n < 2^20)"); return LF_ERR_BAD_ARG; }
    LF_HIP_CHECK(h, hipSetDevice(h->device));
    hipStream_t s = h->stream;
    std::vector<uint32_t> e((size_t)n);
    for (int i = 0; i < n; ++i) {
        if (keys[i] < 0 || keys[i] > 1023) { lf_set_error(h, LF_ERR_BAD_ARG, "lf_debug_std_sort: keys must be in [0, 1023]"); return LF_ERR_BAD_ARG; }
        e[i] = ((uint32_t)keys[i] << 20) | (uint32_t)(i + 1);
    }
    int rc;
    const size_t words = std_sort_debug_words(n);
    Staging st(h);
    const uint32_t* d_e = st.in(0, e.data(), (size_t)n * 4, h->a_q);
    if ((rc = scratch(h, h->a_m, words * 4)) || (rc = scratch(h, h->a_best, 64)) || (rc = st.upload())) return rc;
    launch_std_sort_debug(d_e, static_cast<uint32_t*>(h->a_m.p), n, static_cast<int*>(h->a_best.p), s);
    LF_HIP_CHECK(h, hipGetLastError());
    int cnt = 0;
// ... 121 lines not shown
            if (v == 2) strong[fy * p.Ww + (x >> 5)] |= 1u << (x & 31);
        }
    LF_HIP_CHECK(h, hipSetDevice(h->device));
    hipStream_t s = h->stream;
    DevArray<uint32_t> d_weak, d_strong;
    DevArray<uint8_t> d_edges;
    LF_HIP_CHECK(h, d_weak.alloc(nw * 4));
    LF_HIP_CHECK(h, d_strong.alloc(nw * 4));
    LF_HIP_CHECK(h, d_edges.alloc(npx));
    LF_HIP_CHECK(h, hipMemcpyAsync(d_weak, weak.data(), nw * 4, hipMemcpyHostToDevice, s));
    LF_HIP_CHECK(h, hipMemcpyAsync(d_strong, strong.data(), nw * 4, hipMemcpyHostToDevice, s));
    int rc = LF_OK;
    if (launch_hysteresis(p, n_frames, d_strong, d_weak, s) != 0) {
        lf_set_error(h, LF_ERR_UNSUPPORTED, "img_cols %d: one row of the edge bit planes exceeds the hysteresis strip budget", cols);
        rc = LF_ERR_UNSUPPORTED;
    } else {
        launch_edges_u8(p, n_frames, d_strong, d_edges, s);
        const hipError_t e = hipGetLastError();
        if (e != hipSuccess) { lf_set_error(h, LF_ERR_HIP, "lf_debug_hysteresis: %s", hipGetErrorString(e)); rc = LF_ERR_HIP; }
        else rc = fetch(h, { { edges, d_edges.p, npx } });
    }
    (void)hipStreamSynchronize(s);
    return rc;
}

extern "C" int lf_debug_fetch(lf_handle* h, int buffer_id, void* dst, size_t bytes)
{
    if (!h) return LF_ERR_NOT_INITIALISED;
    if (!dst) { lf_set_error(h, LF_ERR_BAD_ARG, "lf_debug_fetch: null dst"); return LF_ERR_BAD_ARG; }
    LF_HIP_CHECK(h, hipSetDevice(h->device));
    hipStream_t s = h->stream;
    const size_t n = (size_t)h->last_frames;
    const void* src = nullptr;
    size_t avail = 0;
    switch (buffer_id) {
    case LF_BUF_BGR: {
        int rc = scratch(h, h->dbg_bgr, n * h->P * 3);
        if (rc != LF_OK) return rc;
        launch_bgrx_to_bgr((int)(n * h->P), h->d_bgr, (uint8_t*)h->dbg_bgr.p, s);
        src = h->dbg_bgr.p; avail = n * h->P * 3; break;
    }
    case LF_BUF_MASKS: {
        int rc = scratch(h, h->dbg_masks, n * 3 * h->P);
        if (rc != LF_OK) return rc;
        launch_edges_u8(h->canny, (int)(n * 3), h->d_maskbits, (uint8_t*)h->dbg_masks.p, s);
        src = h->dbg_masks.p; avail = n * 3 * h->P; break;
    }
    case LF_BUF_EDGES:
        launch_edges_u8(h->canny, (int)n, h->d_strong, h->d_edges_u8, s);
        src = h->d_edges_u8; avail = n * h->P; break;
    case LF_BUF_LSD_ANGLE:
    case LF_BUF_LSD_MODGRAD: {
        const LsdState& L = h->lsd;
        int rc = scratch(h, h->dbg_ang, n * 3 * L.Ps * sizeof(float));
        if (rc == LF_OK) rc = scratch(h, h->dbg_mod, n * 3 * L.Ps * sizeof(double));
        if (rc != LF_OK) return rc;
        launch_lsd_dense_debug(L.params, L.compact(), (int)n, (float*)h->dbg_ang.p, (double*)h->dbg_mod.p, s);
        if (buffer_id == LF_BUF_LSD_ANGLE) { src = h->dbg_ang.p; avail = n * 3 * L.Ps * sizeof(float); }
        else { src = h->dbg_mod.p; avail = n * 3 * L.Ps * sizeof(double); }
        break;
    }
    case LF_BUF_LSD_ORDER: {
        const size_t row = h->lsd.Ps * sizeof(uint32_t), have = (size_t)h->lsd.params.rec_cap * sizeof(uint32_t);
        if (bytes > n * 3 * row) { lf_set_error(h, LF_ERR_CAPACITY, "buffer %d holds %zu bytes, %zu requested", buffer_id, n * 3 * row, bytes); return LF_ERR_CAPACITY; }
        LF_HIP_CHECK(h, hipMemcpy2DAsync(dst, row, h->lsd.d_order_a, have, have, bytes / row, hipMemcpyDeviceToHost, s));
        LF_HIP_CHECK(h, hipStreamSynchronize(s));
        return LF_OK;
    }
    case LF_BUF_LSD_NORDER: src = h->lsd.d_norder; avail = n * 3 * sizeof(int); break;
    case LF_BUF_LBD_DX:
    case LF_BUF_LBD_DY: {
        int rc = scratch(h, h->dbg_dx, n * h->P * sizeof(int16_t));
        if (rc == LF_OK) rc = scratch(h, h->dbg_dy, n * h->P * sizeof(int16_t));
        if (rc != LF_OK) return rc;
        launch_lbd_split_debug(n * h->P, h->d_dxy, (int16_t*)h->dbg_dx.p, (int16_t*)h->dbg_dy.p, s);
        src = buffer_id == LF_BUF_LBD_DX ? h->dbg_dx.p : h->dbg_dy.p;
        avail = n * h->P * sizeof(int16_t);
        break;
    }
    case LF_BUF_LSD_COUNTS: src = h->d_counts; avail = n * 3 * sizeof(int); break;
    case LF_BUF_LSD_NLOW:
        if (!h->lsd.d_nlow) { memset(dst, 0, bytes < n * 3 * sizeof(int) ? bytes : n * 3 * sizeof(int)); return LF_OK; }
        src = h->lsd.d_nlow; avail = n * 3 * sizeof(int); break;
    case LF_BUF_LSD_SCRATCH: src = h->lsd.d_reg; avail = n * 3 * lsd_grow_reg_stride(h->lsd.params) * sizeof(uint32_t); break;
    default: lf_set_error(h, LF_ERR_BAD_ARG, "unknown buffer id %d", buffer_id); return LF_ERR_BAD_ARG;
    }
    if (bytes > avail) { lf_set_error(h, LF_ERR_CAPACITY, "buffer %d holds %zu bytes, %zu requested", buffer_id, avail, bytes); return LF_ERR_CAPACITY; }
    return fetch(h, { { dst, src, bytes } });
}

extern "C" int lf_debug_assoc_plan(int nq, int nm, int32_t out[6])
{
    if (!out || nq < 1 || nm < 1 || nm > (1 << 21)) return LF_ERR_BAD_ARG;
    const AssocPlan p = assoc_plan(nq, nm);
    out[0] = p.small ? 1 : 0; out[1] = p.qw; out[2] = p.qblocks; out[3] = p.splits; out[4] = p.m_chunk; out[5] = p.nm_pad;
    return LF_OK;
}
```

### lane_slam_amd/csrc/lanefront_handle.h

```cpp
#pragma once
#include <stdio.h>
#include <stdlib.h>
#include <string.h>
#include <memory>
#include <utility>
#include <vector>
#include "lanefront_core.h"
#include "jpeg_entropy.h"
#include "k_edlines_types.h"
#include "k_hough.h"
#include "k_jenc.h"
#include "k_rectify.h"

namespace lf {

struct JpegState {
    lf::jpeg::WorkerPool pool;
    std::vector<lf::jpeg::FrameCoefs> frames;
    int rows = 0, cols = 0, max_frames = 0;
    DevBuf planes, entries, block_end, hdrs, out;
    DevBuf gh_clean, gh_sub, gh_seg, gh_info, gh_coef;
    std::vector<int> h_status;
    HostArray<void> h_stage;
    hipEvent_t staged = nullptr;
// ... 108 lines not shown
    LsdCompact compact() const;
    LsdComponents components(bool use_perm = true) const;
    void grad(int n, const uint32_t* edge_bits, const uint32_t* mask_bits, bool counters_zeroed, hipStream_t s);
    void grad_gray(int n, const uint8_t* gray, hipStream_t s);
    void order(int n, int big, hipStream_t s);
    void label(int n, bool rank, hipStream_t s);
    void grow(int n, float* lines, int* counts, int lds_kb, bool mixed, bool use_perm, hipStream_t s);
};

struct LsdKlLevel {
    LsdState lsd;
    DevArray<float> lines;
    DevArray<int> counts;
    lf_lsd_options opts{};
    bool ready = false;
};

struct LsdKlState {
    LsdKlLevel level[LF_MAX_OCTAVES];
    DevBuf pyr[LF_MAX_OCTAVES];
    KlBatch batch;
};

struct InFlight {
    enum Kind { NONE, SEGMENTS, KEYLINES } kind = NONE;
    const uint8_t* in = nullptr; int n = 0; lf_segments out{}; bool describe = false;
    int problems = 0, capacity = 0;
};

struct MatcherState {
    DevBuf codes;
    std::vector<std::pair<int, int> > index_map;
    int num_images = 0;
    int total = 0;
    DevBuf q, idx, dist, off;
};

}

struct lf_handle : lf::Core {
    lf_config cfg;
    int max_frames = 0, cap_lines = 0;
    int Hc = 0, W = 0, Ww = 0;
    size_t P = 0;
    lf_descriptor_params desc_params = { 1, 7, 2, 5 };
    lf::PreParams pre;
    lf::CannyParams canny;
    lf::LsdState lsd;
    lf::SegParams seg;
    lf::DevArray<uint8_t> d_frames, d_edges_u8;
    lf::DevBuf dbg_masks;
    size_t frames_bytes = 0;
    lf::DevArray<uint32_t> d_bgr;
    lf::DevArray<uint8_t> d_gray;
    lf::DevBuf dbg_bgr;
    lf::DevArray<uint32_t> d_strong, d_weak, d_maskbits;
    lf::DevArray<int> d_sdiv, d_hdiv;
    bool overflow_zeroed = false;
    lf::DevBuf dbg_ang, dbg_mod;
    lf::DevArray<int> d_counts, d_seg_offset, d_frame_offset;
    lf::DevArray<float> d_slot_lines;
    lf::DevArray<int> d_seg_frame;
    lf::DevArray<uint32_t> d_dxy;
    lf::DevBuf dbg_dx, dbg_dy;
    lf::DevArray<float> d_gauss_g, d_gauss_l;
    lf_segments d_out;
    lf::DevArray<float> out_lines, out_normals, out_pixels_normalized;
    lf::DevArray<uint8_t> out_color, out_keep, out_code;
    lf::DevArray<double> out_ground;
    lf::DevArray<float> out_desc;
    lf::DevArray<double> d_normals64;
    lf::DevArray<float> d_centers;
    int out_capacity = 0;
    lf::DevBuf a_q, a_m, a_mx, a_best, a_idx, a_dist, a_qn, a_mn;
    lf::DevBuf km_pts, km_lab, km_f64, km_cnt;
    lf::DevBuf ai_strip, ai_lab, ai_fit, ai_out;
    lf::DevBuf dr_img, dr_fo, dr_lines, dr_color, dr_bad;
    int draw_frames = 0;
    lf::DevBuf kn_hist, kn_count, kn_off, kn_total;
    lf::AssocScratch a_ws;
    std::unique_ptr<lf::MatcherState> matcher;
    lf::HostArray<lf::BatchStatus> h_status;
    lf::InFlight flight;
    int last_frames = 0;
    bool plugin_ready = false;
    lf::HostArray<uint8_t> plug_host, plug_in;
    int plug_eager = 0;
    int detector = LF_DETECTOR_LSD;
    lf_edlines_params ed_params;
    int detector_failures = 0;
    lf_hough_params hough_params = { 2, 3, 1, 1.0, 3.14159265358979323846 / 180 };
    lf::DevArray<lf::HoughTables> d_hough_tab;
    lf::DevArray<int> d_hough_acc;
    lf::DevArray<uint32_t> d_hough_nz;
    lf::HoughParams hough_p{};
    int hough_slots = 0;
    lf_dense_params dense_params = { 40.0 };
    lf::DevArray<uint32_t> d_bwbits;
    lf::DevArray<float> d_dense_rec;
    lf::SegMode slot_mode = lf::SEG_FLOAT;
    int tie_rule = LF_TIE_MIHASHER;
    int env_kl_lds_lines = 0;
    std::vector<int> h_counts, h_seg_offset;
    std::unique_ptr<lf::JpegState> jpeg;
    std::unique_ptr<lf::JencState> jenc;
    std::unique_ptr<lf::RectState> rect;
    std::unique_ptr<lf::KlState> kl;
    std::unique_ptr<lf::LsdKlState> lsdkl;
    lf::DevBuf m_fo, m_color, m_pn, m_nm, m_gr, m_keep, m_counts, m_boff, m_body, m_bad;
    lf::StageClock clock{LF_N_STAGES, 8192, true};
};

namespace lf {

inline bool alloc_trace() { static const bool on = [] { const char* e = getenv("LF_ALLOC_TRACE"); return e && *e && *e != '0'; }(); return on; }
template <typename T>
inline int dalloc_(lf_handle* h, DevArray<T>* p, size_t count, const char* what)
{
    const size_t bytes = count ? count * sizeof(T) : sizeof(T);
    LF_HIP_CHECK(h, p->alloc(bytes));
    if (alloc_trace()) fprintf(stderr, "lanefront alloc %-28s %12zu B\n", what, bytes);
    return LF_OK;
}
#define dalloc(h, p, count) dalloc_(h, p, count, #p)

inline void seg_camera(lf_handle* h)
{
    const lf_config& c = h->cfg;
    SegParams& S = h->seg;
    S.cw = (double)c.cam_w; S.ch = (double)c.cam_h;
    memcpy(S.K, c.K, sizeof(S.K)); memcpy(S.D, c.D, sizeof(S.D));
    for (int i = 0; i < 3; ++i)
        for (int j = 0; j < 3; ++j) {
            double s = 0;
            for (int t = 0; t < 3; ++t) s += c.P[4 * i + t] * c.R[3 * t + j];
            S.RR[3 * i + j] = s;
        }
}

int run_detect(lf_handle* h, const uint8_t* d_frames, int n, bool from_working_image);
int run_segments(lf_handle* h, int n, lf_segments dev_out, bool describe);
inline int refuse_in_flight(lf_handle* h)
{
    if (h->flight.kind != InFlight::NONE) { lf_set_error(h, LF_ERR_BAD_ARG, "a batch is in flight on this handle: call lf_wait first"); return LF_ERR_BAD_ARG; }
    return LF_OK;
}
int plugin_stage_image(lf_handle* h, const uint8_t* bgr, int rows, int cols, int row_stride_bytes);
PreParams plugin_working_pre(const lf_handle* h);
int plugin_finish(lf_handle* h, const uint32_t* mask_bits);
int hough_prepare(lf_handle* h);
int dense_prepare(lf_handle* h);
int run_detect_edlines(lf_handle* h, const uint8_t* d_frames, int n);

}
```

### lane_slam_amd/csrc/lanefront_map.hip

```cpp
#include <stdio.h>
#include <string.h>
#include <new>
#include <vector>
#include "lanefront_map_handle.h"

static char g_map_create_err[512] = "no error";

int refresh_state(lf_map* m, bool block)
{
    if (m->state_pending) {
        if (block) LF_HIP_CHECK(m, hipEventSynchronize(m->ev_state));
        else if (hipEventQuery(m->ev_state) != hipSuccess) return LF_OK;
        m->state_pending = false;
        m->rows_in_flight = 0;
    }
    if (m->h_state[8] != m->errors_reported) {
        const int n_new = m->h_state[8] - m->errors_reported, flags = m->h_state[2];
        m->errors_reported = m->h_state[8];
        if (flags & 2) { set_error(m, LF_ERR_BAD_ARG, "lf_map_update was given a block with a bad header (magic / count): that update was not applied (%d failing update(s) since the last report)", n_new); return LF_ERR_BAD_ARG; }
        if (flags & 4) { set_error(m, LF_ERR_CAPACITY, "a rank's segments did not fit its block (overflow marker in a gathered header): that step's update was applied on no replica (%d failing update(s) since the last report)", n_new); return LF_ERR_CAPACITY; }
        set_error(m, LF_ERR_CAPACITY, "the map is full (capacity %d, LF_MAP_FULL_ERROR): segments were dropped (%d failing update(s) since the last report)", m->cfg.capacity, n_new);
        return LF_ERR_CAPACITY;
    }
    return LF_OK;
// ... 132 lines not shown
    TRY(hipMemsetAsync(m->d.totals, 0, 2 * sizeof(unsigned long long), m->stream));
    launch_fill_i32(m->d.winner, cap, -1, m->stream);
    TRY(hipGetLastError());
    TRY(hipStreamSynchronize(m->stream));
#undef TRY
    m->d.capacity = cfg->capacity; m->d.policy = cfg->policy; m->d.kept_only = cfg->kept_only;
    m->d.merge_distance = cfg->merge_distance; m->d.when_full = cfg->when_full;
    *out = m;
    return LF_OK;
}

extern "C" int lf_map_get_stream(lf_map* m, void** hip_stream)
{
    if (!m) return LF_ERR_NOT_INITIALISED;
    if (!hip_stream) { set_error(m, LF_ERR_BAD_ARG, "lf_map_get_stream: null argument"); return LF_ERR_BAD_ARG; }
    *hip_stream = static_cast<void*>(m->stream);
    return LF_OK;
}

extern "C" int lf_map_synchronize(lf_map* m)
{
    if (!m) return LF_ERR_NOT_INITIALISED;
    LF_HIP_CHECK(m, hipSetDevice(m->device));
    LF_HIP_CHECK(m, hipStreamSynchronize(m->stream));
    return LF_OK;
}

int update_blocks(lf_map* m, const uint8_t* blocks, int n_blocks, int block_rows, int force_append, long long rows_hint)
{
    int rc;
    const size_t rows = (size_t)n_blocks * (size_t)(block_rows - 1);
    if (rows >= (1u << 30)) { set_error(m, LF_ERR_CAPACITY, "lf_map_update: too many rows"); return LF_ERR_CAPACITY; }
    if ((rc = scratch(m, m->act, (rows + rows / 256 + 2) * sizeof(int))) != LF_OK) return rc;
    {
        StageClock::Scope t(m, m->clock, 3);
        launch_map_update(m->d, blocks, n_blocks, block_rows, force_append, static_cast<int*>(m->act.p), m->stream);
    }
    LF_HIP_CHECK(m, hipGetLastError());
    m->rows_in_flight += rows_hint >= 0 ? rows_hint : (long long)rows;
    return queue_state_copy(m);
}

extern "C" int lf_map_update(lf_map* m, const uint8_t* blocks, int n_blocks, int block_rows)
{
    if (!m) return LF_ERR_NOT_INITIALISED;
    if (!blocks || n_blocks < 1 || block_rows < 1) { set_error(m, LF_ERR_BAD_ARG, "lf_map_update: null blocks, n_blocks < 1 or block_rows < 1"); return LF_ERR_BAD_ARG; }
    LF_HIP_CHECK(m, hipSetDevice(m->device));
    if (block_rows == 1) return LF_OK;
    return update_blocks(m, blocks, n_blocks, block_rows, 0);
}

extern "C" int lf_map_seed(lf_map* m, const uint8_t* code32, const uint8_t* color, const double* ground4, int n, int on_device)
{
    if (!m) return LF_ERR_NOT_INITIALISED;
    if (n < 0 || (n > 0 && !code32)) { set_error(m, LF_ERR_BAD_ARG, "lf_map_seed: bad argument"); return LF_ERR_BAD_ARG; }
    if (n == 0) return LF_OK;
    LF_HIP_CHECK(m, hipSetDevice(m->device));
    int rc;
    Staging st(m);
    const uint8_t* dcode = st.in(on_device, code32, (size_t)n * 32, m->seed_code);
    const uint8_t* dcolor = color ? st.in(on_device, color, (size_t)n, m->seed_color) : nullptr;
    const double* dground = ground4 ? st.in(on_device, ground4, (size_t)n * 32, m->seed_ground) : nullptr;
    if ((rc = scratch(m, m->own_block, (size_t)(n + 1) * LF_BLOCK_ROW_BYTES)) || (rc = st.upload())) return rc;
    launch_map_seed_block(n, dcode, dcolor, dground, static_cast<uint8_t*>(m->own_block.p), m->stream);
    rc = update_blocks(m, static_cast<const uint8_t*>(m->own_block.p), 1, n + 1, 1, n);
    if (rc != LF_OK) return rc;
    if (!on_device) LF_HIP_CHECK(m, hipStreamSynchronize(m->stream));
    return LF_OK;
}

extern "C" int lf_map_size(lf_map* m, int* size, int* head, int64_t* total_appended, int64_t* total_refreshed)
{
    if (!m) return LF_ERR_NOT_INITIALISED;
    LF_HIP_CHECK(m, hipSetDevice(m->device));
    const int rc = refresh_state(m);
    if (size) *size = m->h_state[0];
    if (head) *head = m->h_state[1];
    const unsigned long long* t = reinterpret_cast<const unsigned long long*>(m->h_state + 16);
    if (total_appended) *total_appended = (int64_t)t[0];
    if (total_refreshed) *total_refreshed = (int64_t)t[1];
    return rc;
}

extern "C" int lf_map_associate(lf_map* m, lf_handle* h, const uint8_t* code32, const uint8_t* color, int n,
                                int32_t* idx, float* dist, int on_device)
{
    if (!m) return LF_ERR_NOT_INITIALISED;
    if (n < 0 || (n > 0 && (!code32 || !idx || !dist))) { set_error(m, LF_ERR_BAD_ARG, "lf_map_associate: bad argument"); return LF_ERR_BAD_ARG; }
    if (m->cfg.color_gating && n > 0 && !color) { set_error(m, LF_ERR_BAD_ARG, "lf_map_associate: colour gating is on, colours are required"); return LF_ERR_BAD_ARG; }
    if (n == 0) return LF_OK;
    LF_HIP_CHECK(m, hipSetDevice(m->device));
    int rc;
    if ((rc = refresh_state(m, false)) != LF_OK) return rc;
    long long bound = (long long)m->h_state[0] + (m->state_pending ? m->rows_in_flight : 0);
    if (bound > m->cfg.capacity) bound = m->cfg.capacity;
    const int size = (int)bound;
    if (m->tie_rule == LF_TIE_MIHASHER && size > 0 && !assoc_ties_fit(assoc_plan(n, size))) {
        set_error(m, LF_ERR_UNSUPPORTED, "lf_map_associate: %d queries are more than the tie pass of LF_TIE_MIHASHER takes (261888): split the batch or use LF_TIE_LOWEST", n);
        return LF_ERR_UNSUPPORTED;
    }
    if ((rc = after_handle(m, h)) != LF_OK) return rc;
    hipStream_t s = m->stream;
    Staging st(m);
    const uint8_t* dq = st.in(on_device, code32, (size_t)n * 32, m->q_in);
    const uint8_t* dc = color ? st.in(on_device, color, (size_t)n, m->c_in) : nullptr;
    int32_t* didx = st.out(on_device, idx, (size_t)n * 4, m->idx_out);
    float* ddist = st.out(on_device, dist, (size_t)n * 4, m->dist_out);
    if (m->tie_rule == LF_TIE_MIHASHER && (rc = scratch(m, m->tie_res, (size_t)n * 8)) != LF_OK) return rc;
    if ((rc = st.upload()) != LF_OK) return rc;
    if (size == 0) {
        launch_assoc_nomatch(n, didx, ddist, s);
    } else {
        {
            StageClock::Scope t(m, m->clock, 1);
            m->ws.tie_res = m->tie_rule == LF_TIE_MIHASHER ? static_cast<unsigned long long*>(m->tie_res.p) : nullptr;
            LF_HIP_CHECK(m, launch_assoc_core(dq, m->cfg.color_gating ? dc : nullptr, n, m->d.mx, m->d.mcx, size, m->d.state, m->cfg.color_gating,
                                         m->cfg.max_distance, m->ws, didx, ddist, s));
            if (m->tie_rule == LF_TIE_MIHASHER)
                LF_HIP_CHECK(m, launch_assoc_ties(dq, m->cfg.color_gating ? dc : nullptr, n, m->d.mx, m->d.code, m->d.color, size, m->d.state,
                                             m->cfg.color_gating, m->ws, static_cast<unsigned long long*>(m->tie_res.p), didx, ddist, s));
        }
    }
    LF_HIP_CHECK(m, hipGetLastError());
    if ((rc = release_handle(m, h)) != LF_OK) return rc;
    return fetch(m, { { idx, didx, (size_t)n * 4 }, { dist, ddist, (size_t)n * 4 } });
}

extern "C" int lf_map_set_tie_rule(lf_map* m, int tie_rule)
{
    if (!m) return LF_ERR_NOT_INITIALISED;
    if (tie_rule != LF_TIE_LOWEST && tie_rule != LF_TIE_MIHASHER) { set_error(m, LF_ERR_BAD_ARG, "lf_map_set_tie_rule: unknown rule"); return LF_ERR_BAD_ARG; }
    m->tie_rule = tie_rule;
    return LF_OK;
}

extern "C" int lf_map_pack_block(lf_map* m, lf_handle* h, const lf_segments* segs, int n, int n_frames, const int32_t* idx,
                                 const float* dist, const double* frame_pose, int step, uint8_t* block, int block_rows)
{
    if (!m) return LF_ERR_NOT_INITIALISED;
    if (!segs || !block || n < 0 || (n > 0 && !segs->code) || (frame_pose && (n_frames < 1 || !segs->frame_offset))) {
        set_error(m, LF_ERR_BAD_ARG, "lf_map_pack_block: bad argument (segs->code is required; frame_pose needs segs->frame_offset and n_frames >= 1)");
        return LF_ERR_BAD_ARG;
    }
    if (block_rows < 1) { set_error(m, LF_ERR_BAD_ARG, "lf_map_pack_block: block_rows < 1"); return LF_ERR_BAD_ARG; }
    LF_HIP_CHECK(m, hipSetDevice(m->device));
    int rc;
    if (n + 1 > block_rows) {
        launch_map_overflow_block(n, n_frames, step, block, m->stream);
        LF_HIP_CHECK(m, hipGetLastError());
        set_error(m, LF_ERR_CAPACITY, "lf_map_pack_block: %d segments do not fit a block of %d rows (header + %d); only a header with the overflow marker was written", n, block_rows, block_rows - 1);
        return LF_ERR_CAPACITY;
    }
    if ((rc = after_handle(m, h)) != LF_OK) return rc;
    const double* dpose = nullptr;
    if (frame_pose) {
        m->h_pose.resize((size_t)n_frames * 4);
        for (int f = 0; f < n_frames; ++f) {
            double sn, cs;
            dm::dsincos(frame_pose[3 * f + 2], sn, cs);
            m->h_pose[4 * f] = frame_pose[3 * f]; m->h_pose[4 * f + 1] = frame_pose[3 * f + 1];
            m->h_pose[4 * f + 2] = cs; m->h_pose[4 * f + 3] = sn;
        }
        if ((rc = scratch(m, m->pose, (size_t)n_frames * 4 * sizeof(double))) != LF_OK) return rc;
        LF_HIP_CHECK(m, hipMemcpyAsync(m->pose.p, m->h_pose.data(), (size_t)n_frames * 4 * sizeof(double), hipMemcpyHostToDevice, m->stream));
        dpose = static_cast<const double*>(m->pose.p);
    }
    {
        StageClock::Scope t(m, m->clock, 2);
        launch_map_pack_block(n, n_frames, segs->frame_offset, segs->code, segs->color, segs->keep, segs->ground, idx, dist, dpose, step,
                              block, m->stream);
    }
    LF_HIP_CHECK(m, hipGetLastError());
    return release_handle(m, h);
}

extern "C" int lf_map_step(lf_map* m, lf_handle* h, const lf_segments* segs, int n, int n_frames, const double* frame_pose,
                           int step, int32_t* idx, float* dist)
{
    if (!m) return LF_ERR_NOT_INITIALISED;
    if (!segs || n < 0 || (n > 0 && (!idx || !dist))) { set_error(m, LF_ERR_BAD_ARG, "lf_map_step: bad argument"); return LF_ERR_BAD_ARG; }
    int rc;
    if ((rc = associate_for_step(m, h, "lf_map_step", segs, n, n_frames, frame_pose, idx, dist)) != LF_OK) return rc;
    LF_HIP_CHECK(m, hipSetDevice(m->device));
    if ((rc = scratch(m, m->own_block, (size_t)(n + 1) * LF_BLOCK_ROW_BYTES)) != LF_OK) return rc;
    if ((rc = lf_map_pack_block(m, h, segs, n, n_frames, idx, dist, frame_pose, step, static_cast<uint8_t*>(m->own_block.p), n + 1)) != LF_OK) return rc;
    if (n == 0) return LF_OK;
    return update_blocks(m, static_cast<const uint8_t*>(m->own_block.p), 1, n + 1, 0, n);
}

extern "C" int lf_map_step_host(lf_map* m, const lf_segments* segs, int n, int n_frames, const double* frame_pose, int step,
                                int32_t* idx, float* dist)
{
    if (!m) return LF_ERR_NOT_INITIALISED;
    if (!segs || n < 0 || n_frames < 1 || (n > 0 && (!segs->code || !idx || !dist)) || !segs->frame_offset ||
        (m->cfg.color_gating && n > 0 && !segs->color)) {
        set_error(m, LF_ERR_BAD_ARG, "lf_map_step_host: bad argument (frame_offset and code are required, color when gating is on)");
        return LF_ERR_BAD_ARG;
    }
    return step_from_host(m, segs, n, n_frames, idx, dist, [&](const lf_segments* d, int32_t* d_idx, float* d_dist) {
        return lf_map_step(m, nullptr, d, n, n_frames, frame_pose, step, d_idx, d_dist);
    });
}

extern "C" int lf_map_fetch(lf_map* m, int first, int n, uint8_t* code32, uint8_t* color, double* ground4, int32_t* hits,
                            int32_t* last_seen)
{
    if (!m) return LF_ERR_NOT_INITIALISED;
    if (first < 0 || n < 0 || (long long)first + n > m->cfg.capacity) { set_error(m, LF_ERR_BAD_ARG, "lf_map_fetch: range [%d, %d) outside the map's capacity %d", first, first + n, m->cfg.capacity); return LF_ERR_BAD_ARG; }
    LF_HIP_CHECK(m, hipSetDevice(m->device));
    const size_t f = (size_t)first, c = (size_t)n;
    return fetch(m, { { code32, m->d.code + f * 32, c * 32 }, { color, m->d.color + f, c }, { ground4, m->d.ground + f * 4, c * 32 },
                      { hits, m->d.hits + f, c * 4 }, { last_seen, m->d.last_seen + f, c * 4 } });
}
```

### lane_slam_amd/csrc/lanefront_map_handle.h

```cpp
#pragma once
#include <functional>
#include <memory>
#include <vector>
#include "lanefront_core.h"
#include "k_map_align.h"
#include "k_map_near.h"
#include "k_map_polylines.h"

namespace lf {

struct MapNearState {
    DevBuf start, cursor, bucket, rec, pose, near_out;
    std::vector<double> h_pose;
};

struct MapLanesState {
    DevBuf work, counters, lane_of, n_links, support, lanes;
    HostArray<int> h_counters;
};

struct MapPolylinesState {
    DevBuf lanes_work, lanes_counters, lane_of;
    DevBuf work, counters, vertex_of, vertices, polylines;
    HostArray<int> h_counters;
};

struct MapLanePoseState {
    DevBuf vertices, polylines, edges, pose, out;
    std::vector<double> h_pose;
};

struct MapRenderState {
    DevBuf px, tiles, list, traj, counters, bounds, out;
    HostArray<int> h_counters;
    int n_drawn = 0, n_skipped = 0;
    bool rendered = false;
    CallClock clock{LF_MAP_RENDER_STAGES};
    hipEvent_t done = nullptr;
    ~MapRenderState()
    {
        if (done) (void)hipEventDestroy(done);
    }
};

struct MapCameraState {
    DevBuf tiles, rec, pose, counters, frames;
    HostArray<int> h_counters;
    std::vector<double> h_pose;
    bool rendered = false;
    CallClock clock{LF_MAP_RENDER_STAGES};
};

struct MapPruneState {
    DevBuf reason, rank, wg, counters, rec, s_code, s_color, s_ground, s_hits, s_last, remap;
    HostArray<int> h_counters;
};

struct MapGraphState {
    DevBuf in, work, keys;
    std::vector<uint8_t> h_in, h_keys;
    std::vector<double> h_out;
};

}

using namespace lf;

enum MapStage {
    kMapAlignStage = LF_MAP_N_STAGES, kMapSmoothStage, kMapLocalizeStage, kMapPruneStage,
    kMapNearIndexStage, kMapNearQueryStage,
    kMapLanesIndexStage, kMapLanesTableStage,
    kMapPolylinesLanesStage, kMapPolylinesVerticesStage, kMapPolylinesLinksStage,
    kMapLanePosePolylinesStage, kMapLanePoseQueryStage,
    kMapGraphSolveStage, kMapCorrectStage,
    kMapStageCount
};

struct lf_map : lf::Core {
    lf_map_config cfg;
    int tie_rule = LF_TIE_MIHASHER;
    MapDevice d;
    DevArray<uint8_t> code, color;
    DevArray<double> ground;
    DevArray<int> hits, last_seen, winner, state;
    DevArray<int8_t> mx, mcx;
    DevArray<unsigned long long> totals;
    size_t cap_pad = 0;
    HostArray<int> h_state;
    int errors_reported = 0;
    hipEvent_t ev_state = nullptr, ev_in = nullptr, ev_out = nullptr;
    bool state_pending = false;
    long long rows_in_flight = 0;
    AssocScratch ws;
    DevBuf act, own_block, pose, q_in, c_in, idx_out, dist_out, seed_code, seed_color, seed_ground, tie_res;
    DevBuf st_fo, st_code, st_color, st_keep, st_ground, st_idx, st_dist;
    DevBuf prior_pose;
    DevBuf al_res;
    DevBuf sm_offset, sm_chain_of, sm_sums, sm_node, sm_chain, sm_status;
    DevBuf lo_res;
    std::vector<double> h_pose;
    std::vector<int32_t> h_chains;
    StageClock clock{kMapStageCount, 4096, false};
    bool near_on = false;
    lf_near_config near_cfg = {};
    std::unique_ptr<lf::MapNearState> near;
    std::unique_ptr<lf::MapLanesState> lanes;
    std::unique_ptr<lf::MapPolylinesState> polylines;
    std::unique_ptr<lf::MapLanePoseState> lane_pose;
    std::unique_ptr<lf::MapGraphState> graph;
    std::unique_ptr<lf::MapPruneState> prune;
    std::unique_ptr<lf::MapRenderState> render;
    std::unique_ptr<lf::MapCameraState> camera;
};

int refresh_state(lf_map* m, bool block = true);
int queue_state_copy(lf_map* m);
int after_handle(lf_map* m, lf_handle* h);
int release_handle(lf_map* m, lf_handle* h);
int update_blocks(lf_map* m, const uint8_t* blocks, int n_blocks, int block_rows, int force_append, long long rows_hint = -1);
int settled_size(lf_map* m, size_t* size);
int take_stages(lf_map* m, int first, int n, double* ms, int32_t* launches);

int build_index(lf_map* m, size_t bound, double cell, int stage, nr::Index* ix);

constexpr int kTailCounters = 8;
constexpr int kPolylinesCounters = ln::kNCounters + pl::kNCounters + kTailCounters;
const char* polylines_bad_config(const lf_polylines_config* c);
lf::MapPolylinesState& polylines_state(lf_map* m);
int queue_polylines(lf_map* m, const lf_polylines_config* c, size_t bound, const pl::Out& o, const int* stages, int** counters);
int polylines_result(lf_map* m, const char* who, size_t bound, lf_polylines_result* res);

int associate_for_step(lf_map* m, lf_handle* h, const char* who, const lf_segments* segs, int n, int n_frames, const double* frame_pose,
                       int32_t* idx, float* dist);

int solver_check_call(lf_map* m, const char* who, const lf_segments* segs, int n, int n_frames, const int32_t* idx, const double* pose,
                      bool pose_required, bool has_cfg, const void* results);
int align_check_call(lf_map* m, const char* who, const lf_segments* segs, int n, int n_frames, const int32_t* idx, const double* frame_pose,
                     const lf_align_config* cfg, const void* results);
ma::Batch batch_view(const lf_segments* d, int n, int n_frames, const int32_t* idx, const float* dist);
int open_batch(lf_map* m, lf_handle* h, const lf_segments* segs, int n, int n_frames, const int32_t* idx, const float* dist, int on_device,
               ma::Batch* b);
int upload_prior_pose(lf_map* m, const double* pose, int n_frames, const double** d_pose);

int step_solved(lf_map* m, lf_handle* h, const char* who, const lf_segments* segs, int n, int n_frames, const double* frame_pose, int step,
                int32_t* idx, float* dist,
                const std::function<int(const ma::Batch&)>& queue_solver);
int step_from_host(lf_map* m, const lf_segments* segs, int n, int n_frames, int32_t* idx, float* dist,
                   const std::function<int(const lf_segments* d, int32_t* d_idx, float* d_dist)>& device_form);
```

### lane_slam_amd/frontend.py

```python
import ctypes

import numpy as np

from . import _lib
from .config import LfConfig, default_config, fill_struct, work_size


class LanefrontError(RuntimeError):
    def __init__(self, code, msg):
        RuntimeError.__init__(self, "lanefront error %d: %s" % (code, msg))
        self.code = code


class Segments(object):

    __slots__ = ("n", "frame_offset", "lines", "normals", "color", "pixels_normalized", "ground", "keep",
                 "desc", "code")

    def frame(self, f):
        a, b = int(self.frame_offset[f]), int(self.frame_offset[f + 1])
        out = Segments()
        out.n = b - a
        out.frame_offset = np.array([0, b - a], np.int32)
        for k in ("lines", "normals", "color", "pixels_normalized", "ground", "keep", "desc", "code"):
# ... 513 lines not shown
        ang = np.ascontiguousarray(angle, np.float32)
        npx = np.ascontiguousarray(num_pixels, np.int32)
        octv = np.ascontiguousarray(octave, np.int32)
        n = io.shape[0]
        desc, code = np.zeros((n, 72), np.float32), np.zeros((n, 32), np.uint8)
        self._check(self.lib.lf_describe_keylines(self.h, _ptr(gray), gray.shape[0], _ptr(fr), _ptr(io), _ptr(ang), _ptr(npx), _ptr(octv), n,
                                                  _ptr(desc), _ptr(code), 0))
        return desc, code

    def keylines_fetch(self, octave, what, n_frames):
        dims = np.zeros(5, np.int32)
        self._check(self.lib.lf_keylines_debug_fetch(self.h, int(octave), int(what), None, 0, _ptr(dims)))
        H, W, cap, max_edges, max_lines = (int(v) for v in dims)
        shape, dt = {0: ((H, W), np.uint8), 1: ((H, W), np.uint32), 2: ((H, W), np.uint16), 3: ((cap,), np.uint32), 4: ((2 * cap,), np.uint32),
                     5: ((max_edges + 2,), np.uint32), 6: ((4,), np.int32), 7: ((max_lines, 4), np.float32), 8: ((max_lines,), np.float64),
                     9: ((max_lines,), np.float32), 10: ((max_lines,), np.int32), 11: ((max_lines,), np.float32), 12: ((H, W), np.uint8)}[what]
        a = np.empty((n_frames,) + shape, dt)
        self._check(self.lib.lf_keylines_debug_fetch(self.h, int(octave), int(what), _ptr(a), a.nbytes, None))
        return a

    def decode_jpeg_batch(self, streams, rows=None, cols=None, n_threads=0, device_ptr=None, entropy="gpu"):
        n = len(streams)
        rows = self.cfg["in_size"][0] if rows is None else rows
        cols = self.cfg["in_size"][1] if cols is None else cols
        keep = [b if isinstance(b, bytes) else bytes(b) for b in streams]
        ptrs = ctypes.cast((ctypes.c_char_p * n)(*[b if len(b) else None for b in keep]), ctypes.POINTER(ctypes.c_void_p))
        sizes = (ctypes.c_size_t * n)(*[len(b) for b in keep])
        status = np.zeros(n, np.int32)
        st = status.ctypes.data_as(ctypes.POINTER(ctypes.c_int))
        if entropy not in ("gpu", "host"):
            raise ValueError("entropy must be 'gpu' or 'host'")
        fn = self.lib.lf_jpeg_decode_batch_gpu if entropy == "gpu" else self.lib.lf_jpeg_decode_batch
        if device_ptr is None:
            out = np.empty((n, rows, cols, 3), np.uint8)
            self._check(fn(self.h, ptrs, sizes, n, rows, cols, _ptr(out), 0, n_threads, st))
            return out, status
        self._check(fn(self.h, ptrs, sizes, n, rows, cols, ctypes.c_void_p(int(device_ptr)), 1, n_threads, st))
        return status

    def decode_jpeg_batch_async(self, streams, device_ptr=None, rows=None, cols=None, n_threads=0, for_detect=False):
        n = len(streams)
        rows = self.cfg["in_size"][0] if rows is None else rows
        cols = self.cfg["in_size"][1] if cols is None else cols
        own = self.frames_buffer()[0]
        if device_ptr is None:
            device_ptr = own
        keep = [b if isinstance(b, bytes) else bytes(b) for b in streams]
        ptrs = ctypes.cast((ctypes.c_char_p * n)(*[b if len(b) else None for b in keep]), ctypes.POINTER(ctypes.c_void_p))
        sizes = (ctypes.c_size_t * n)(*[len(b) for b in keep])
        if for_detect:
            if int(device_ptr) != own or (rows, cols) != tuple(self.cfg["in_size"]):
                raise ValueError("for_detect decodes frames of the configured size into the handle's own buffer")
            self._check(self.lib.lf_jpeg_decode_for_detect_async(self.h, ptrs, sizes, n, n_threads))
        else:
            self._check(self.lib.lf_jpeg_decode_batch_gpu_async(self.h, ptrs, sizes, n, rows, cols, ctypes.c_void_p(int(device_ptr)), n_threads))
        self._jpeg_queued = n
        return int(device_ptr)

    def jpeg_status(self):
        n = getattr(self, "_jpeg_queued", 0)
        status = np.zeros(n, np.int32)
        self._check(self.lib.lf_jpeg_status(self.h, status.ctypes.data_as(ctypes.POINTER(ctypes.c_int)), n, None))
        return status

    def frames_buffer(self):
        p, nb = ctypes.c_void_p(), ctypes.c_size_t()
        self._check(self.lib.lf_frames_buffer(self.h, ctypes.byref(p), ctypes.byref(nb)))
        return p.value, nb.value

    def fetch(self, buffer_id, n_frames):
        P, Ps = self.rows * self.cols, self.lsd_rows * self.lsd_cols
        shapes = {
            _lib.LF_BUF_BGR: ((n_frames, self.rows, self.cols, 3), np.uint8),
            _lib.LF_BUF_MASKS: ((n_frames, 3, self.rows, self.cols), np.uint8),
            _lib.LF_BUF_EDGES: ((n_frames, self.rows, self.cols), np.uint8),
            _lib.LF_BUF_LSD_ANGLE: ((n_frames, 3, self.lsd_rows, self.lsd_cols), np.float32),
            _lib.LF_BUF_LSD_MODGRAD: ((n_frames, 3, self.lsd_rows, self.lsd_cols), np.float64),
            _lib.LF_BUF_LSD_ORDER: ((n_frames, 3, Ps), np.uint32),
            _lib.LF_BUF_LSD_NORDER: ((n_frames, 3), np.int32),
            _lib.LF_BUF_LBD_DX: ((n_frames, self.rows, self.cols), np.int16),
            _lib.LF_BUF_LBD_DY: ((n_frames, self.rows, self.cols), np.int16),
            _lib.LF_BUF_LSD_COUNTS: ((n_frames, 3), np.int32),
            _lib.LF_BUF_LSD_NLOW: ((n_frames, 3), np.int32),
            _lib.LF_BUF_LSD_SCRATCH: ((n_frames, 3, int(self.lib.lf_lsd_scratch_stride(self.h))), np.uint32),
        }
        shape, dt = shapes[buffer_id]
        a = np.empty(shape, dt)
        self._check(self.lib.lf_debug_fetch(self.h, buffer_id, _ptr(a), a.nbytes))
        return a

    def lsd_binary(self, img, cap=8192):
        img = np.ascontiguousarray(img, dtype=np.uint8)
        lines = np.empty((cap, 4), np.float32)
        n = ctypes.c_int()
        self._check(self.lib.lf_debug_lsd_binary(self.h, _ptr(img), img.shape[0], img.shape[1], _ptr(lines), cap, ctypes.byref(n)))
        return lines[:n.value].copy()

    def debug_hysteresis(self, planes):
        planes = np.ascontiguousarray(planes, dtype=np.uint8)
        p3 = planes[None] if planes.ndim == 2 else planes
        if p3.ndim != 3:
            raise ValueError("planes must be (n, rows, cols) or (rows, cols), got %r" % (planes.shape,))
        edges = np.empty(p3.shape, np.uint8)
        self._check(self.lib.lf_debug_hysteresis(self.h, _ptr(p3), p3.shape[0], p3.shape[1], p3.shape[2], _ptr(edges)))
        return edges.reshape(planes.shape)

    def debug_segments(self, counts, lines, masks=None, mode="float", out=None, capacity=None):
        counts = np.ascontiguousarray(counts, dtype=np.int32).reshape(-1, 3)
        n = counts.shape[0]
        lines = np.ascontiguousarray(lines, dtype=np.float32)
        if lines.size != n * 3 * self.cap_lines * 4:
            raise ValueError("lines must be (%d, 3, %d, 4), got %r" % (n, self.cap_lines, lines.shape))
        if masks is not None:
            masks = np.ascontiguousarray(masks, dtype=np.uint8)
            if masks.shape != (n, 3, self.rows, self.cols):
                raise ValueError("masks must be (%d, 3, %d, %d), got %r" % (n, self.rows, self.cols, masks.shape))
        cap = n * 3 * self.cap_lines if capacity is None else int(capacity)
        if out is None:
            out = {"frame_offset": np.zeros(n + 1, np.int32), "lines": np.empty((cap, 4), np.float32), "normals": np.empty((cap, 2), np.float32),
                   "color": np.empty(cap, np.uint8), "pixels_normalized": np.empty((cap, 4), np.float32),
                   "ground": np.empty((cap, 4), np.float64), "keep": np.empty(cap, np.uint8)}
        s = _lib.LfSegments()
        s.capacity = cap
        for k, v in out.items():
            setattr(s, k, v.ctypes.data)
        total = ctypes.c_int(-1)
        rc = self.lib.lf_debug_segments(self.h, {"float": 0, "hough": 1}.get(mode, mode), n, _ptr(counts), _ptr(lines),
                                        None if masks is None else _ptr(masks), ctypes.byref(s), ctypes.byref(total))
        if rc != 0:
            e = LanefrontError(rc, self.lib.lf_last_error(self.h).decode())
            e.n_segments = total.value
            raise e
        seg = Segments()
        seg.n = total.value
        seg.frame_offset = out.get("frame_offset")
        for k in ("lines", "normals", "color", "pixels_normalized", "ground", "keep"):
            setattr(seg, k, out[k][:seg.n] if k in out else None)
        seg.desc = seg.code = None
        return seg

    def set_profiling(self, on):
        self._check(self.lib.lf_set_profiling(self.h, int(bool(on))))

    def reset_timing(self):
        self._check(self.lib.lf_reset_timing(self.h))

    def timing(self):
        ms = np.zeros(_lib.LF_N_STAGES, np.float64)
        ln = np.zeros(_lib.LF_N_STAGES, np.int32)
        self._check(self.lib.lf_get_timing(self.h, _ptr(ms), _ptr(ln), _lib.LF_N_STAGES))
        return {self.lib.lf_stage_name(i).decode(): (float(ms[i]), int(ln[i])) for i in range(_lib.LF_N_STAGES)}
```

### lane_slam_amd/line_associator.py

```python
import collections
import ctypes

import numpy as np

from . import _lib

BLOCK_ROW_BYTES = 80
_POLICY = {"append": 0, "merge": 1}
_WHEN_FULL = {"ring": 0, "error": 1}
Lanes = collections.namedtuple("Lanes", ("result", "lane_of", "n_links", "support", "lanes"))
LANE_BYTES = ctypes.sizeof(_lib.LfLane)
Polylines = collections.namedtuple("Polylines", ("result", "vertex_of", "vertices", "polylines"))
POLYLINE_VERTEX_BYTES = ctypes.sizeof(_lib.LfPolylineVertex)
POLYLINE_BYTES = ctypes.sizeof(_lib.LfPolyline)
LANE_POSE_BYTES = ctypes.sizeof(_lib.LfMapLanePose)


class LineAssociator(object):
    def __init__(self, capacity=65536, color_gating=False, max_distance=128, policy="append", kept_only=True,
                 merge_distance=0, when_full="ring", device=0, tie_rule=None):
        self.lib = _lib.load()
        if tie_rule is not None and tie_rule not in _lib.TIE_RULES:
            raise ValueError("tie_rule must be one of %r" % (sorted(_lib.TIE_RULES),))
        if policy not in _POLICY or when_full not in _WHEN_FULL:
            raise ValueError("policy must be 'append' or 'merge', when_full 'ring' or 'error'")
        self.capacity = int(capacity)
        self._device = int(device)
        self.color_gating = bool(color_gating)
        c = _lib.LfMapConfig(self.capacity, int(self.color_gating), int(max_distance), _POLICY[policy], int(bool(kept_only)),
                             int(merge_distance), _WHEN_FULL[when_full])
        self.m = ctypes.c_void_p()
        rc = self.lib.lf_map_create(int(device), ctypes.byref(c), ctypes.byref(self.m))
        if rc != 0:
            msg = self.lib.lf_map_last_error(None).decode()
            self.m = None
            from .frontend import LanefrontError
            raise LanefrontError(rc, msg)
        if tie_rule is not None:
            self._check(self.lib.lf_map_set_tie_rule(self.m, _lib.TIE_RULES[tie_rule]))

    def close(self):
        if getattr(self, "m", None):
            self.lib.lf_map_destroy(self.m)
            self.m = None

    def __del__(self):
        try:
            self.close()
        except Exception:
            pass

    def _check(self, rc):
        if rc != 0:
            from .frontend import LanefrontError
            raise LanefrontError(rc, self.lib.lf_map_last_error(self.m).decode())

    def stream_ptr(self):
        p = ctypes.c_void_p()
        self._check(self.lib.lf_map_get_stream(self.m, ctypes.byref(p)))
        return p.value or 0

    def synchronize(self):
        self._check(self.lib.lf_map_synchronize(self.m))

    def set_profiling(self, on):
        self._check(self.lib.lf_map_set_profiling(self.m, int(bool(on))))

    def timing(self):
        ms = np.zeros(_lib.LF_MAP_N_STAGES, np.float64)
        ln = np.zeros(_lib.LF_MAP_N_STAGES, np.int32)
        self._check(self.lib.lf_map_get_timing(self.m, ms.ctypes.data, ln.ctypes.data, _lib.LF_MAP_N_STAGES))
        return {self.lib.lf_map_stage_name(i).decode(): (float(ms[i]), int(ln[i])) for i in range(_lib.LF_MAP_N_STAGES)}

    def seed(self, codes, colors=None, ground=None):
        codes = np.ascontiguousarray(codes, np.uint8).reshape(-1, 32)
        colors = None if colors is None else np.ascontiguousarray(colors, np.uint8)
        ground = None if ground is None else np.ascontiguousarray(ground, np.float64).reshape(-1, 4)
        self._check(self.lib.lf_map_seed(self.m, codes.ctypes.data, None if colors is None else colors.ctypes.data,
                                         None if ground is None else ground.ctypes.data, codes.shape[0], 0))

    def seed_device(self, code_ptr, n, color_ptr=None, ground_ptr=None):
        self._check(self.lib.lf_map_seed(self.m, int(code_ptr), color_ptr and int(color_ptr), ground_ptr and int(ground_ptr), int(n), 1))

    def state(self):
        size, head = ctypes.c_int(), ctypes.c_int()
        ta, tr = ctypes.c_int64(), ctypes.c_int64()
        self._check(self.lib.lf_map_size(self.m, ctypes.byref(size), ctypes.byref(head), ctypes.byref(ta), ctypes.byref(tr)))
        return {"size": size.value, "head": head.value, "total_appended": ta.value, "total_refreshed": tr.value}

    def associate(self, codes, colors=None):
        codes = np.ascontiguousarray(codes, np.uint8).reshape(-1, 32)
        colors = None if colors is None else np.ascontiguousarray(colors, np.uint8)
        n = codes.shape[0]
        idx, dist = np.empty(n, np.int32), np.empty(n, np.float32)
        self._check(self.lib.lf_map_associate(self.m, None, codes.ctypes.data, None if colors is None else colors.ctypes.data, n,
                                              idx.ctypes.data, dist.ctypes.data, 0))
        return idx, dist

    def step(self, seg, poses=None, step=0, align=None, smooth=None, chains=None):
        if align is not None and smooth is not None:
            raise ValueError("step: align and smooth exclude each other")
        n, n_frames = int(seg.n), len(seg.frame_offset) - 1
        keep_alive, pp = self._poses(poses, n_frames)
        s, alive = self._host_segs(seg, ("frame_offset", "code", "color", "keep", "ground"))
        idx, dist = np.empty(n, np.int32), np.empty(n, np.float32)
        if align is None and smooth is None:
            self._check(self.lib.lf_map_step_host(self.m, ctypes.byref(s), n, n_frames, pp, int(step), idx.ctypes.data, dist.ctypes.data))
            return idx, dist
        res = np.zeros(n_frames, _lib.ALIGN_RESULT_DTYPE)
        if smooth is not None:
            co, cp, nc = self._chains(chains, n_frames)
            self._check(self.lib.lf_map_step_smoothed_host(self.m, ctypes.byref(s), n, n_frames, pp, cp, nc, ctypes.byref(smooth), int(step),
                                                           idx.ctypes.data, dist.ctypes.data, res.ctypes.data, None))
            return idx, dist, self._poses_out(res), res
        self._check(self.lib.lf_map_step_aligned_host(self.m, ctypes.byref(s), n, n_frames, pp, ctypes.byref(align), int(step),
                                                      idx.ctypes.data, dist.ctypes.data, res.ctypes.data))
        return idx, dist, self._poses_out(res), res

    @staticmethod
    def _host_segs(seg, keys):
        s = _lib.LfSegments()
        s.capacity = int(seg.n)
        alive = []
        for k in keys:
            v = getattr(seg, k, None)
            if v is not None:
                a = np.ascontiguousarray(v)
                alive.append(a)
                setattr(s, k, a.ctypes.data)
        return s, alive

    def _config(self, who, kind, default, overrides, nested=None):
        c = kind()
        default(ctypes.byref(c))
        if nested is not None and nested[1] is not None:
            ctypes.memmove(ctypes.byref(getattr(c, nested[0])), ctypes.byref(nested[1]), ctypes.sizeof(nested[1]))
        own = dict((k, t) for k, t in kind._fields_ if k != "reserved_" and (nested is None or k != nested[0]))
        inner = {} if nested is None else dict((k, t) for k, t in type(getattr(c, nested[0]))._fields_)
        for k, val in overrides.items():
            if k in own:
                setattr(c, k, int(val) if own[k] is ctypes.c_int32 else float(val))
            elif k in inner:
                setattr(getattr(c, nested[0]), k, int(val) if inner[k] is ctypes.c_int32 else float(val))
            else:
                raise TypeError("%s: unknown field %r" % (who, k))
        return c

    def _solver_host(self, who, seg, idx, dist, poses):
        n, n_frames = int(seg.n), len(seg.frame_offset) - 1
        keep_alive, pp = self._poses(poses, n_frames)
        s, alive = self._host_segs(seg, ("frame_offset", "color", "keep", "ground"))
        idx = np.ascontiguousarray(idx, np.int32)
        dist = None if dist is None else np.ascontiguousarray(dist, np.float32)
        if len(idx) != n or (dist is not None and len(dist) != n):
            raise ValueError("%s: idx and dist hold one value per segment" % who)
# ... 586 lines not shown
```

Baseline: 117,700.

## Snapshot batch outputs for map association and parallelize LSD rank kernel

When association runs on device outputs from the last processed batch, the segment arrays are copied into map-owned scratch with one fused kernel, and the handle is released early. A later pack_block on the same batch reads that copy instead of waiting on the handle, so the next frontend batch can overlap with the map stages. Separately, the LSD rank kernel moves from a single 256-thread block (which fell back to identity above 1024 entries) to a multi-block tiled rank over int4 shared tiles, which scales to larger problems. The change adds snapshot bookkeeping counters, new debug buffer IDs, and an extra device copy per associate call.

```diff
diff --git a/include/lanefront.h b/include/lanefront.h
--- a/include/lanefront.h
+++ b/include/lanefront.h
@@ -172,6 +172,7 @@
 LF_API int lf_map_size(lf_map* m, int* size, int* head, int64_t* total_appended, int64_t* total_refreshed);
 LF_API int lf_map_associate(lf_map* m, lf_handle* h, const uint8_t* code32, const uint8_t* color, int n,
                      int32_t* idx, float* dist, int on_device);
+LF_API int lf_map_snapshot_counts(lf_map* m, int64_t* taken, int64_t* reused, int64_t* fallback);
 LF_API int lf_map_set_tie_rule(lf_map* m, int tie_rule);
 LF_API int lf_map_pack_block(lf_map* m, lf_handle* h, const lf_segments* segs, int n, int n_frames, const int32_t* idx,
                       const float* dist, const double* frame_pose, int step, uint8_t* block, int block_rows);
@@ -604,7 +605,9 @@
     LF_BUF_LBD_DY = 8,
     LF_BUF_LSD_COUNTS = 9,
     LF_BUF_LSD_SCRATCH = 10,
-    LF_BUF_LSD_NLOW = 11
+    LF_BUF_LSD_NLOW = 11,
+    LF_BUF_LSD_COMP_KEY = 12,
+    LF_BUF_LSD_PERM = 13
 } lf_buffer_id;
 LF_API int lf_debug_fetch(lf_handle* h, int buffer_id, void* dst, size_t bytes);
 LF_API int lf_debug_detmath(lf_handle* h, int which, const double* a, const double* b_or_null, double* y, int n);
diff --git a/lane_slam_amd/_lib.py b/lane_slam_amd/_lib.py
--- a/lane_slam_amd/_lib.py
+++ b/lane_slam_amd/_lib.py
@@ -10,7 +10,8 @@
 LF_MAP_N_STAGES = 4
 LF_MSG_DETECTOR, LF_MSG_GROUND, LF_MSG_FILTERED = 0, 1, 2
 (LF_BUF_BGR, LF_BUF_MASKS, LF_BUF_EDGES, LF_BUF_LSD_ANGLE, LF_BUF_LSD_MODGRAD, LF_BUF_LSD_ORDER,
- LF_BUF_LSD_NORDER, LF_BUF_LBD_DX, LF_BUF_LBD_DY, LF_BUF_LSD_COUNTS, LF_BUF_LSD_SCRATCH, LF_BUF_LSD_NLOW) = range(12)
+ LF_BUF_LSD_NORDER, LF_BUF_LBD_DX, LF_BUF_LBD_DY, LF_BUF_LSD_COUNTS, LF_BUF_LSD_SCRATCH, LF_BUF_LSD_NLOW,
+ LF_BUF_LSD_COMP_KEY, LF_BUF_LSD_PERM) = range(14)
 
 EXPORTS = (
     "lf_abi_version", "lf_create", "lf_destroy", "lf_last_error", "lf_synchronize", "lf_get_stream",
@@ -19,7 +20,7 @@
     "lf_debug_fetch", "lf_debug_detmath", "lf_debug_wave", "lf_debug_probe", "lf_debug_lsd_binary", "lf_debug_segments", "lf_debug_hysteresis", "lf_lsd_size", "lf_set_profiling", "lf_get_timing", "lf_reset_timing", "lf_stage_name",
     "lf_map_create", "lf_map_destroy", "lf_map_last_error", "lf_map_get_stream", "lf_map_synchronize", "lf_map_seed", "lf_map_size",
     "lf_map_associate", "lf_map_pack_block", "lf_map_update", "lf_map_step", "lf_map_step_host", "lf_map_fetch",
-    "lf_map_set_profiling", "lf_map_get_timing", "lf_map_stage_name",
+    "lf_map_set_profiling", "lf_map_get_timing", "lf_map_stage_name", "lf_map_snapshot_counts",
     "lf_descriptor_default_params", "lf_set_descriptor_params", "lf_get_descriptor_params",
     "lf_edlines_default_params", "lf_keylines_batch", "lf_describe_keylines", "lf_keylines_debug_fetch", "lf_set_image_edlines", "lf_knn_match", "lf_radius_match", "lf_jpeg_decode_batch_gpu", "lf_jpeg_decode_batch_gpu_async", "lf_jpeg_status", "lf_jpeg_decode_for_detect_async",
     "lf_set_tie_rule", "lf_map_set_tie_rule", "lf_debug_std_sort", "lf_debug_assoc_plan", "lf_suggested_depth", "lf_lsd_list_capacity", "lf_lsd_scratch_stride", "lf_set_detector", "lf_detector_failures", "lf_keylines_batch_async", "lf_keylines_frame_status", "lf_lsd_keylines_batch", "lf_select_queries",
@@ -397,6 +398,8 @@
     lib.lf_map_get_timing.restype = ci
     lib.lf_map_stage_name.argtypes = [ci]
     lib.lf_map_stage_name.restype = ctypes.c_char_p
+    lib.lf_map_snapshot_counts.argtypes = [vp, i64p, i64p, i64p]
+    lib.lf_map_snapshot_counts.restype = ci
     lib.lf_map_default_view.argtypes = [ctypes.POINTER(LfMapView)]
     lib.lf_map_default_view.restype = None
     lib.lf_map_bounds.argtypes = [vp, ctypes.POINTER(LfMapView), vp, ctypes.POINTER(ci)]
diff --git a/lane_slam_amd/csrc/common.h b/lane_slam_amd/csrc/common.h
--- a/lane_slam_amd/csrc/common.h
+++ b/lane_slam_amd/csrc/common.h
@@ -329,6 +329,15 @@
                            const uint8_t* keep, const double* ground, const int32_t* idx, const float* dist,
                            const double* pose4, int step, uint8_t* block, hipStream_t s);
 void launch_map_overflow_block(int n, int n_frames, int step, uint8_t* block, hipStream_t s);
+constexpr int kSnapshotArrays = 5;
+struct MapSnapshotCopy {
+    const uint8_t* src[kSnapshotArrays];
+    uint8_t* dst[kSnapshotArrays];
+    uint32_t bytes[kSnapshotArrays];
+    uint32_t end16[kSnapshotArrays];
+};
+bool map_snapshot_plan(MapSnapshotCopy* c);
+void launch_map_snapshot(const MapSnapshotCopy& c, hipStream_t s);
 void launch_map_seed_block(int n, const uint8_t* code, const uint8_t* color, const double* ground, uint8_t* block, hipStream_t s);
 void launch_map_update(const MapDevice& md, const uint8_t* blocks, int n_blocks, int block_rows, int force_append, int* act,
                        hipStream_t s);
diff --git a/lane_slam_amd/csrc/k_lsd_order.hip b/lane_slam_amd/csrc/k_lsd_order.hip
--- a/lane_slam_amd/csrc/k_lsd_order.hip
+++ b/lane_slam_amd/csrc/k_lsd_order.hip
@@ -607,26 +607,48 @@
     }
 }
 
-__global__ __launch_bounds__(256) void k_lsd_rank(int n_prob, const int* __restrict__ norder, int* __restrict__ perm)
-{
-    __shared__ int nd[1024];
-    if (n_prob > 1024) {
-        for (int i = threadIdx.x; i < n_prob; i += 256) perm[i] = i;
-        return;
-    }
-    for (int i = threadIdx.x; i < n_prob; i += 256) nd[i] = norder[i];
-    __syncthreads();
-    for (int i = threadIdx.x; i < n_prob; i += 256) {
-        const int mine = nd[i];
-        int rank = 0;
-        for (int j = 0; j < n_prob; ++j) rank += (nd[j] > mine || (nd[j] == mine && j < i)) ? 1 : 0;
-        perm[rank] = i;
-    }
+constexpr int kRankTile = 1024, kRankWave = 64;
+__global__ __launch_bounds__(kRankWave) void k_lsd_rank(int n_prob, const int* __restrict__ norder, int* __restrict__ perm)
+{
+    __shared__ int4 nd[kRankTile / 4];
+    const int i = blockIdx.x * kRankWave + threadIdx.x;
+    const int mine = i < n_prob ? norder[i] : 0;
+    int rank = 0;
+    for (int base = 0; base < n_prob; base += kRankTile) {
+        const int m = min(kRankTile, n_prob - base);
+        const int nq = ((m + 31) / 32) * 8;
+        if (base) __syncthreads();
+        for (int q = threadIdx.x; q < nq; q += kRankWave) {
+            const int j = base + 4 * q;
+            int4 v;
+            if (j + 4 <= n_prob) v = *reinterpret_cast<const int4*>(norder + j);
+            else {
+                v.x = j < n_prob ? norder[j] : INT_MIN;
+                v.y = j + 1 < n_prob ? norder[j + 1] : INT_MIN;
+                v.z = j + 2 < n_prob ? norder[j + 2] : INT_MIN;
+                v.w = INT_MIN;
+            }
+            nd[q] = v;
+        }
+        __syncthreads();
+        const int before = i - base;
+#pragma unroll 8
+        for (int q = 0; q < nq; ++q) {
+            const int4 v = nd[q];
+            const int j = 4 * q;
+            rank += (v.x > mine || (v.x == mine && j < before)) ? 1 : 0;
+            rank += (v.y > mine || (v.y == mine && j + 1 < before)) ? 1 : 0;
+            rank += (v.z > mine || (v.z == mine && j + 2 < before)) ? 1 : 0;
+            rank += (v.w > mine || (v.w == mine && j + 3 < before)) ? 1 : 0;
+        }
+    }
+    if (i < n_prob) perm[rank] = i;
 }
 
 void launch_lsd_rank(const LsdComponents& m, int n_prob, hipStream_t s)
 {
-    hipLaunchKernelGGL(k_lsd_rank, dim3(1), dim3(256), 0, s, n_prob, m.comp_key, m.perm);
+    if (n_prob < 1) return;
+    hipLaunchKernelGGL(k_lsd_rank, dim3((n_prob + kRankWave - 1) / kRankWave), dim3(kRankWave), 0, s, n_prob, m.comp_key, m.perm);
 }
 
 __global__ __launch_bounds__(LT) void k_lsd_label(LsdParams p, const int* __restrict__ norder, const uint32_t* __restrict__ c_xy,
diff --git a/lane_slam_amd/csrc/k_map.hip b/lane_slam_amd/csrc/k_map.hip
--- a/lane_slam_amd/csrc/k_map.hip
+++ b/lane_slam_amd/csrc/k_map.hip
@@ -232,6 +232,42 @@
                        keep, ground, idx, dist, pose4, step, block);
 }
 
+__global__ __launch_bounds__(256) void k_map_snapshot(MapSnapshotCopy c)
+{
+    const uint32_t t = blockIdx.x * 256u + threadIdx.x;
+    const uint8_t* src = nullptr;
+    uint8_t* dst = nullptr;
+    uint32_t bytes = 0, first = 0, begin = 0;
+#pragma unroll
+    for (int k = 0; k < kSnapshotArrays; ++k) {
+        if (t >= begin && t < c.end16[k]) { src = c.src[k]; dst = c.dst[k]; bytes = c.bytes[k]; first = begin; }
+        begin = c.end16[k];
+    }
+    if (!src) return;
+    const uint32_t o = (t - first) * 16u;
+    if (o + 16u <= bytes) *reinterpret_cast<uint4*>(dst + o) = *reinterpret_cast<const uint4*>(src + o);
+    else for (uint32_t b = o; b < bytes; ++b) dst[b] = src[b];
+}
+
+bool map_snapshot_plan(MapSnapshotCopy* c)
+{
+    unsigned long long end = 0;
+    for (int k = 0; k < kSnapshotArrays; ++k) {
+        if (!c->src[k]) c->bytes[k] = 0;
+        if (c->bytes[k] && ((reinterpret_cast<uintptr_t>(c->src[k]) | reinterpret_cast<uintptr_t>(c->dst[k])) & 15u)) return false;
+        end += (c->bytes[k] + 15ull) / 16;
+        if (end >= (1ull << 31)) return false;
+        c->end16[k] = (uint32_t)end;
+    }
+    return true;
+}
+
+void launch_map_snapshot(const MapSnapshotCopy& c, hipStream_t s)
+{
+    const uint32_t threads = c.end16[kSnapshotArrays - 1];
+    if (threads) hipLaunchKernelGGL(k_map_snapshot, dim3((threads + 255) / 256), dim3(256), 0, s, c);
+}
+
 __global__ void k_map_overflow_block(int n, int n_frames, int step, uint8_t* __restrict__ block)
 {
     uint32_t* hd = reinterpret_cast<uint32_t*>(block);
diff --git a/lane_slam_amd/csrc/lanefront_api.hip b/lane_slam_amd/csrc/lanefront_api.hip
--- a/lane_slam_amd/csrc/lanefront_api.hip
+++ b/lane_slam_amd/csrc/lanefront_api.hip
@@ -2,6 +2,7 @@
 #include <stdio.h>
 #include <string.h>
 #include <math.h>
+#include <atomic>
 #include <vector>
 #include <new>
 #include <cstdlib>
@@ -366,6 +367,10 @@
 
 static int fetch_status(lf_handle* h) { LF_HIP_CHECK(h, hipMemcpyAsync(h->h_status, h->lsd.d_status, sizeof(BatchStatus), hipMemcpyDeviceToHost, h->stream)); return LF_OK; }
 
+static std::atomic<unsigned long long> g_batch_serial{0};
+
+LastBatch lf::last_batch_of(const lf_handle* h) { return h ? h->last_batch : LastBatch{}; }
+
 extern "C" int lf_process_batch_async(lf_handle* h, const uint8_t* frames, int n_frames, int frames_on_device,
                                       lf_segments* out_dev, int describe)
 {
@@ -388,6 +393,7 @@
         d_in = h->d_frames;
     }
     h->plugin_ready = false;
+    h->last_batch = LastBatch{ *out_dev, n_frames, g_batch_serial.fetch_add(1, std::memory_order_relaxed) + 1 };
     int rc = h->detector == LF_DETECTOR_EDLINES ? run_detect_edlines(h, d_in, n_frames) : run_detect(h, d_in, n_frames, false);
     if (rc != LF_OK) return rc;
     rc = run_segments(h, n_frames, *out_dev, describe != 0);
diff --git a/lane_slam_amd/csrc/lanefront_core.h b/lane_slam_amd/csrc/lanefront_core.h
--- a/lane_slam_amd/csrc/lanefront_core.h
+++ b/lane_slam_amd/csrc/lanefront_core.h
@@ -124,6 +124,13 @@
     LF_HIP_CHECK(c, hipStreamWaitEvent(waits, ev, 0));
     return LF_OK;
 }
+
+struct LastBatch {
+    lf_segments out{};
+    int n_frames = 0;
+    unsigned long long serial = 0;
+};
+LastBatch last_batch_of(const lf_handle* h);
 
 struct StageClock {
     struct Rec { hipEvent_t a, b; int st; };
diff --git a/lane_slam_amd/csrc/lanefront_debug.hip b/lane_slam_amd/csrc/lanefront_debug.hip
--- a/lane_slam_amd/csrc/lanefront_debug.hip
+++ b/lane_slam_amd/csrc/lanefront_debug.hip
@@ -227,6 +227,8 @@
     case LF_BUF_LSD_NLOW:
         if (!h->lsd.d_nlow) { memset(dst, 0, bytes < n * 3 * sizeof(int) ? bytes : n * 3 * sizeof(int)); return LF_OK; }
         src = h->lsd.d_nlow; avail = n * 3 * sizeof(int); break;
+    case LF_BUF_LSD_COMP_KEY: src = h->lsd.d_comp_key; avail = n * 3 * sizeof(int); break;
+    case LF_BUF_LSD_PERM: src = h->lsd.d_perm; avail = n * 3 * sizeof(int); break;
     case LF_BUF_LSD_SCRATCH: src = h->lsd.d_reg; avail = n * 3 * lsd_grow_reg_stride(h->lsd.params) * sizeof(uint32_t); break;
     default: lf_set_error(h, LF_ERR_BAD_ARG, "unknown buffer id %d", buffer_id); return LF_ERR_BAD_ARG;
     }
diff --git a/lane_slam_amd/csrc/lanefront_handle.h b/lane_slam_amd/csrc/lanefront_handle.h
--- a/lane_slam_amd/csrc/lanefront_handle.h
+++ b/lane_slam_amd/csrc/lanefront_handle.h
@@ -214,6 +214,7 @@
     std::unique_ptr<lf::MatcherState> matcher;
     lf::HostArray<lf::BatchStatus> h_status;
     lf::InFlight flight;
+    lf::LastBatch last_batch;
     int last_frames = 0;
     bool plugin_ready = false;
     lf::HostArray<uint8_t> plug_host, plug_in;
diff --git a/lane_slam_amd/csrc/lanefront_map.hip b/lane_slam_amd/csrc/lanefront_map.hip
--- a/lane_slam_amd/csrc/lanefront_map.hip
+++ b/lane_slam_amd/csrc/lanefront_map.hip
@@ -238,6 +238,75 @@
     return rc;
 }
 
+constexpr int kSnapshotRows = 16384;
+
+static bool snapshot_applies(const LastBatch& lb, const uint8_t* code32, const uint8_t* color, int n)
+{
+    return lb.serial != 0 && lb.out.code && code32 == lb.out.code && (!color || color == lb.out.color) && n <= lb.out.capacity &&
+           lb.n_frames >= 1 && (size_t)n * 32 < ((size_t)1 << 31);
+}
+
+static int take_snapshot(lf_map* m, lf_handle* h, const LastBatch& lb, int n, bool* taken)
+{
+    *taken = false;
+    MapSnapshot& sp = m->snap;
+    sp.h = nullptr;
+    const int floor_rows = lb.out.capacity < kSnapshotRows ? lb.out.capacity : kSnapshotRows;
+    const size_t rows = (size_t)(n > floor_rows ? n : floor_rows), r16 = (rows + 15) & ~(size_t)15;
+    const size_t fo_bytes = lb.out.frame_offset ? ((size_t)lb.n_frames + 1) * sizeof(int) : 0;
+    if (const int rc = scratch(m, sp.buf, r16 * 66 + ((fo_bytes + 15) & ~(size_t)15))) return rc;
+    uint8_t* base = static_cast<uint8_t*>(sp.buf.p);
+    const size_t sn = (size_t)n;
+    MapSnapshotCopy c = {};
+    const void* src[kSnapshotArrays] = { lb.out.code, lb.out.ground, lb.out.color, lb.out.keep, lb.out.frame_offset };
+    const size_t bytes[kSnapshotArrays] = { sn * 32, sn * 32, sn, sn, fo_bytes };
+    const size_t at[kSnapshotArrays] = { 0, r16 * 32, r16 * 64, r16 * 65, r16 * 66 };
+    for (int k = 0; k < kSnapshotArrays; ++k) {
+        c.src[k] = static_cast<const uint8_t*>(src[k]);
+        c.dst[k] = base + at[k];
+        c.bytes[k] = (uint32_t)bytes[k];
+    }
+    if (!map_snapshot_plan(&c)) return LF_OK;
+    launch_map_snapshot(c, m->stream);
+    LF_HIP_CHECK(m, hipGetLastError());
+    sp.h = h; sp.serial = lb.serial; sp.n = n; sp.n_frames = lb.n_frames; sp.user = lb.out;
+    sp.copy = lf_segments{};
+    sp.copy.capacity = n;
+    sp.copy.code = lb.out.code ? c.dst[0] : nullptr;
+    sp.copy.ground = lb.out.ground ? reinterpret_cast<double*>(c.dst[1]) : nullptr;
+    sp.copy.color = lb.out.color ? c.dst[2] : nullptr;
+    sp.copy.keep = lb.out.keep ? c.dst[3] : nullptr;
+    sp.copy.frame_offset = lb.out.frame_offset ? reinterpret_cast<int32_t*>(c.dst[4]) : nullptr;
+    *taken = true;
+    return LF_OK;
+}
+
+static bool snapshot_serves(const lf_map* m, const lf_handle* h, const lf_segments* segs, int n, int n_frames, bool needs_frames, lf_segments* d)
+{
+    const MapSnapshot& sp = m->snap;
+    if (!h || sp.h != h || last_batch_of(h).serial != sp.serial || n != sp.n || n < 1) return false;
+    if (segs->code != sp.user.code) return false;
+    if ((segs->color && segs->color != sp.user.color) || (segs->keep && segs->keep != sp.user.keep) ||
+        (segs->ground && segs->ground != sp.user.ground) || (segs->frame_offset && segs->frame_offset != sp.user.frame_offset)) return false;
+    if (needs_frames && n_frames > sp.n_frames) return false;
+    *d = lf_segments{};
+    d->code = sp.copy.code;
+    d->color = segs->color ? sp.copy.color : nullptr;
+    d->keep = segs->keep ? sp.copy.keep : nullptr;
+    d->ground = segs->ground ? sp.copy.ground : nullptr;
+    d->frame_offset = segs->frame_offset ? sp.copy.frame_offset : nullptr;
+    return true;
+}
+
+extern "C" int lf_map_snapshot_counts(lf_map* m, int64_t* taken, int64_t* reused, int64_t* fallback)
+{
+    if (!m) return LF_ERR_NOT_INITIALISED;
+    if (taken) *taken = m->snap.taken;
+    if (reused) *reused = m->snap.reused;
+    if (fallback) *fallback = m->snap.fallback;
+    return LF_OK;
+}
+
 extern "C" int lf_map_associate(lf_map* m, lf_handle* h, const uint8_t* code32, const uint8_t* color, int n,
                                 int32_t* idx, float* dist, int on_device)
 {
@@ -257,9 +326,16 @@
     }
     if ((rc = after_handle(m, h)) != LF_OK) return rc;
     hipStream_t s = m->stream;
+    bool snapped = false;
+    if (h && on_device) {
+        const LastBatch lb = last_batch_of(h);
+        if (snapshot_applies(lb, code32, color, n) && (rc = take_snapshot(m, h, lb, n, &snapped)) != LF_OK) return rc;
+        if (snapped && (rc = release_handle(m, h)) != LF_OK) return rc;
+        ++(snapped ? m->snap.taken : m->snap.fallback);
+    }
     Staging st(m);
-    const uint8_t* dq = st.in(on_device, code32, (size_t)n * 32, m->q_in);
-    const uint8_t* dc = color ? st.in(on_device, color, (size_t)n, m->c_in) : nullptr;
+    const uint8_t* dq = snapped ? m->snap.copy.code : st.in(on_device, code32, (size_t)n * 32, m->q_in);
+    const uint8_t* dc = !color ? nullptr : snapped ? m->snap.copy.color : st.in(on_device, color, (size_t)n, m->c_in);
     int32_t* didx = st.out(on_device, idx, (size_t)n * 4, m->idx_out);
     float* ddist = st.out(on_device, dist, (size_t)n * 4, m->dist_out);
     if (m->tie_rule == LF_TIE_MIHASHER && (rc = scratch(m, m->tie_res, (size_t)n * 8)) != LF_OK) return rc;
@@ -278,7 +354,7 @@
         }
     }
     LF_HIP_CHECK(m, hipGetLastError());
-    if ((rc = release_handle(m, h)) != LF_OK) return rc;
+    if (!snapped && (rc = release_handle(m, h)) != LF_OK) return rc;
     return fetch(m, { { idx, didx, (size_t)n * 4 }, { dist, ddist, (size_t)n * 4 } });
 }
 
@@ -307,7 +383,10 @@
         set_error(m, LF_ERR_CAPACITY, "lf_map_pack_block: %d segments do not fit a block of %d rows (header + %d); only a header with the overflow marker was written", n, block_rows, block_rows - 1);
         return LF_ERR_CAPACITY;
     }
-    if ((rc = after_handle(m, h)) != LF_OK) return rc;
+    lf_segments d = *segs;
+    const bool snapped = snapshot_serves(m, h, segs, n, n_frames, frame_pose && segs->frame_offset, &d);
+    if (h) ++(snapped ? m->snap.reused : m->snap.fallback);
+    if (!snapped && (rc = after_handle(m, h)) != LF_OK) return rc;
     const double* dpose = nullptr;
     if (frame_pose) {
         m->h_pose.resize((size_t)n_frames * 4);
@@ -323,11 +402,10 @@
     }
     {
         StageClock::Scope t(m, m->clock, 2);
-        launch_map_pack_block(n, n_frames, segs->frame_offset, segs->code, segs->color, segs->keep, segs->ground, idx, dist, dpose, step,
-                              block, m->stream);
+        launch_map_pack_block(n, n_frames, d.frame_offset, d.code, d.color, d.keep, d.ground, idx, dist, dpose, step, block, m->stream);
     }
     LF_HIP_CHECK(m, hipGetLastError());
-    return release_handle(m, h);
+    return snapped ? LF_OK : release_handle(m, h);
 }
 
 extern "C" int lf_map_step(lf_map* m, lf_handle* h, const lf_segments* segs, int n, int n_frames, const double* frame_pose,
diff --git a/lane_slam_amd/csrc/lanefront_map_handle.h b/lane_slam_amd/csrc/lanefront_map_handle.h
--- a/lane_slam_amd/csrc/lanefront_map_handle.h
+++ b/lane_slam_amd/csrc/lanefront_map_handle.h
@@ -62,6 +62,15 @@
     std::vector<double> h_out;
 };
 
+struct MapSnapshot {
+    DevBuf buf;
+    const lf_handle* h = nullptr;
+    unsigned long long serial = 0;
+    int n = 0, n_frames = 0;
+    lf_segments user{}, copy{};
+    long long taken = 0, reused = 0, fallback = 0;
+};
+
 }
 
 using namespace lf;
@@ -94,6 +103,7 @@
     AssocScratch ws;
     DevBuf act, own_block, pose, q_in, c_in, idx_out, dist_out, seed_code, seed_color, seed_ground, tie_res;
     DevBuf st_fo, st_code, st_color, st_keep, st_ground, st_idx, st_dist;
+    lf::MapSnapshot snap;
     DevBuf prior_pose;
     DevBuf al_res;
     DevBuf sm_offset, sm_chain_of, sm_sums, sm_node, sm_chain, sm_status;
diff --git a/lane_slam_amd/frontend.py b/lane_slam_amd/frontend.py
--- a/lane_slam_amd/frontend.py
+++ b/lane_slam_amd/frontend.py
@@ -619,6 +619,8 @@
             _lib.LF_BUF_LBD_DY: ((n_frames, self.rows, self.cols), np.int16),
             _lib.LF_BUF_LSD_COUNTS: ((n_frames, 3), np.int32),
             _lib.LF_BUF_LSD_NLOW: ((n_frames, 3), np.int32),
+            _lib.LF_BUF_LSD_COMP_KEY: ((n_frames, 3), np.int32),
+            _lib.LF_BUF_LSD_PERM: ((n_frames, 3), np.int32),
             _lib.LF_BUF_LSD_SCRATCH: ((n_frames, 3, int(self.lib.lf_lsd_scratch_stride(self.h))), np.uint32),
         }
         shape, dt = shapes[buffer_id]
diff --git a/lane_slam_amd/line_associator.py b/lane_slam_amd/line_associator.py
--- a/lane_slam_amd/line_associator.py
+++ b/lane_slam_amd/line_associator.py
@@ -71,6 +71,11 @@
         ln = np.zeros(_lib.LF_MAP_N_STAGES, np.int32)
         self._check(self.lib.lf_map_get_timing(self.m, ms.ctypes.data, ln.ctypes.data, _lib.LF_MAP_N_STAGES))
         return {self.lib.lf_map_stage_name(i).decode(): (float(ms[i]), int(ln[i])) for i in range(_lib.LF_MAP_N_STAGES)}
+
+    def snapshot_counts(self):
+        t, r, f = ctypes.c_int64(), ctypes.c_int64(), ctypes.c_int64()
+        self._check(self.lib.lf_map_snapshot_counts(self.m, ctypes.byref(t), ctypes.byref(r), ctypes.byref(f)))
+        return {"taken": t.value, "reused": r.value, "fallback": f.value}
 
     def seed(self, codes, colors=None, ground=None):
         codes = np.ascontiguousarray(codes, np.uint8).reshape(-1, 32)
```

Result: faster. 121,700, median of 6 (+3.4%).
